# microsoft/msrflute

Hardware: AMD Instinct MI355X
Metric: fl_rounds_per_sec (higher is better)
Workload: dtype fp32; 1 GPU; model=cnn_femnist (2conv+2fc, 62 classes), global_batch=200, seq_len=784, parallelism=client-parallel fedavg, 1 ranks, clients=3400, clients_per_round=10, samples_per_client=200, local_epochs=1, client_batch_size=20, eval_and_checkpoint=outside timed region, precision_detail=fp32 throughout

## Files before the change

msrflute_amd/csrc/bindings.cpp:

```cpp

#include <torch/extension.h>
#include <c10/hip/HIPStream.h>
#include <hip/hip_runtime.h>

#include "launchers.h"

namespace {

hipStream_t cur_stream() {
  return c10::hip::getCurrentHIPStream().stream();
}

void check_flat(const torch::Tensor& t, const char* name) {
  TORCH_CHECK(t.is_cuda(), name, " must be on GPU");
  TORCH_CHECK(t.is_contiguous(), name, " must be contiguous");
  TORCH_CHECK(t.scalar_type() == torch::kFloat32, name, " must be fp32");
}

void pseudo_grad(torch::Tensor out, torch::Tensor ws, torch::Tensor wt,
                 double weight) {
  check_flat(out, "out"); check_flat(ws, "ws"); check_flat(wt, "wt");
  TORCH_CHECK(out.numel() == ws.numel() && ws.numel() == wt.numel());
  launch_pseudo_grad(out.data_ptr<float>(), ws.data_ptr<float>(),
                     wt.data_ptr<float>(), (float)weight, out.numel(),
                     cur_stream());
}

void axpy(torch::Tensor y, torch::Tensor x, double alpha) {
  check_flat(y, "y"); check_flat(x, "x");
  TORCH_CHECK(y.numel() == x.numel());
  launch_axpy(y.data_ptr<float>(), x.data_ptr<float>(), (float)alpha,
              y.numel(), cur_stream());
}

void scale(torch::Tensor x, double alpha) {
  check_flat(x, "x");
  launch_scale(x.data_ptr<float>(), (float)alpha, x.numel(), cur_stream());
}

static torch::Tensor sum_sumsq_acc(const torch::Tensor& x) {
  auto acc = torch::zeros({2}, x.options().dtype(torch::kFloat64));
  int nparts = sum_sumsq2_partials(x.numel());
  auto partials = torch::empty({2 * (long long)nparts},
                               x.options().dtype(torch::kFloat64));
  launch_sum_sumsq2(x.data_ptr<float>(), x.numel(),
                    partials.data_ptr<double>(), acc.data_ptr<double>(),
                    cur_stream());
  return acc;
}

torch::Tensor sum_sumsq(torch::Tensor x) {
  check_flat(x, "x");
  return sum_sumsq_acc(x).to(torch::kFloat32);
}

torch::Tensor clip_by_norm(torch::Tensor x, double max_norm, double eps) {
  check_flat(x, "x");
  auto acc = sum_sumsq_acc(x);
  auto norm = torch::empty({}, x.options());
  launch_clip_apply(x.data_ptr<float>(), x.numel(), acc.data_ptr<double>(),
                    (float)max_norm, (float)eps, norm.data_ptr<float>(),
                    cur_stream());
  return norm;
}

void add_gaussian_noise(torch::Tensor x, double sigma, int64_t seed,
                        int64_t offset) {
  check_flat(x, "x");
  launch_add_gaussian_noise(x.data_ptr<float>(), x.numel(), (float)sigma,
                            (unsigned long long)seed,
                            (unsigned long long)offset, cur_stream());
}

void sgd_step(torch::Tensor p, torch::Tensor g, torch::Tensor buf, double lr,
              double momentum, double dampening, double weight_decay,
              bool nesterov, bool first_step) {
  check_flat(p, "p"); check_flat(g, "g");
  if (momentum != 0.0) {
    check_flat(buf, "buf");
    TORCH_CHECK(buf.numel() == p.numel(), "momentum buffer size mismatch");
  }
  launch_sgd_step(p.data_ptr<float>(), g.data_ptr<float>(),
                  buf.numel() ? buf.data_ptr<float>() : nullptr, (float)lr,
                  nullptr, (float)momentum, (float)dampening,
                  (float)weight_decay, nesterov ? 1 : 0, first_step ? 1 : 0,
                  p.numel(), cur_stream());
}

void sgd_step_devlr(torch::Tensor p, torch::Tensor g, torch::Tensor buf,
                    torch::Tensor lr_t, double momentum, double dampening,
                    double weight_decay, bool nesterov, bool first_step) {
  check_flat(p, "p"); check_flat(g, "g"); check_flat(lr_t, "lr_t");
  if (momentum != 0.0) {
    check_flat(buf, "buf");
    TORCH_CHECK(buf.numel() == p.numel(), "momentum buffer size mismatch");
  }
  launch_sgd_step(p.data_ptr<float>(), g.data_ptr<float>(),
                  buf.numel() ? buf.data_ptr<float>() : nullptr, 0.f,
                  lr_t.data_ptr<float>(), (float)momentum, (float)dampening,
                  (float)weight_decay, nesterov ? 1 : 0, first_step ? 1 : 0,
                  p.numel(), cur_stream());
}

void clip_stats_accumulate(torch::Tensor x, double max_norm, double eps,
                           torch::Tensor stats_acc) {
  check_flat(x, "x"); check_flat(stats_acc, "stats_acc");
  TORCH_CHECK(stats_acc.numel() >= 2, "stats_acc must have 2 elements");
  auto acc = sum_sumsq_acc(x);
  launch_clip_apply_stats(x.data_ptr<float>(), x.numel(),
                          acc.data_ptr<double>(), (float)max_norm, (float)eps,
                          stats_acc.data_ptr<float>(), cur_stream());
}

void adam_step(torch::Tensor p, torch::Tensor g, torch::Tensor m,
               torch::Tensor v, torch::Tensor vmax, int64_t step, double lr,
               double beta1, double beta2, double eps, double weight_decay,
               bool amsgrad, bool adamw) {
  check_flat(p, "p"); check_flat(g, "g"); check_flat(m, "m"); check_flat(v, "v");
  if (amsgrad) check_flat(vmax, "vmax");
  float bc1 = 1.0f - (float)std::pow(beta1, (double)step);
  float bc2 = 1.0f - (float)std::pow(beta2, (double)step);
  launch_adam_step(p.data_ptr<float>(), g.data_ptr<float>(),
                   m.data_ptr<float>(), v.data_ptr<float>(),
                   vmax.numel() ? vmax.data_ptr<float>() : nullptr, (float)lr,
                   (float)beta1, (float)beta2, (float)eps, (float)weight_decay,
                   bc1, bc2, amsgrad ? 1 : 0, adamw ? 1 : 0, p.numel(),
                   cur_stream());
}

void adamax_step(torch::Tensor p, torch::Tensor g, torch::Tensor m,
                 torch::Tensor u, int64_t step, double lr, double beta1,
                 double beta2, double eps, double weight_decay) {
  check_flat(p, "p"); check_flat(g, "g"); check_flat(m, "m"); check_flat(u, "u");
  float bc1 = 1.0f - (float)std::pow(beta1, (double)step);
  launch_adamax_step(p.data_ptr<float>(), g.data_ptr<float>(),
                     m.data_ptr<float>(), u.data_ptr<float>(), (float)lr,
                     (float)beta1, (float)beta2, (float)eps,
                     (float)weight_decay, bc1, p.numel(), cur_stream());
}

torch::Tensor segmented_sqnorm(torch::Tensor x, torch::Tensor seg_offsets) {
  check_flat(x, "x");
  TORCH_CHECK(seg_offsets.is_cuda() && seg_offsets.is_contiguous() &&
              seg_offsets.scalar_type() == torch::kInt64,
              "seg_offsets must be contiguous int64 on GPU");
  int n_segs = (int)seg_offsets.numel() - 1;
  auto out = torch::zeros({n_segs}, x.options().dtype(torch::kFloat64));
  launch_segmented_sqnorm(
      x.data_ptr<float>(),
      reinterpret_cast<const long long*>(seg_offsets.data_ptr<int64_t>()),
      n_segs, out.data_ptr<double>(), cur_stream());
  return out.to(torch::kFloat32);
}

void quant_bin_mask(torch::Tensor x, torch::Tensor min_t, torch::Tensor max_t,
                    torch::Tensor thresh_t, int64_t n_bins) {
  check_flat(x, "x");
  check_flat(min_t, "min_t"); check_flat(max_t, "max_t");
  check_flat(thresh_t, "thresh_t");
  launch_quant_bin_mask(x.data_ptr<float>(), x.numel(),
                        min_t.data_ptr<float>(), max_t.data_ptr<float>(),
                        thresh_t.data_ptr<float>(), (int)n_bins, cur_stream());
}

static CnnWorkspace slice_ws(torch::Tensor& work_f, torch::Tensor& work_i,
                             torch::Tensor& work_b, torch::Tensor& work_d,
                             int B, int C) {
  float* f = work_f.data_ptr<float>();
  CnnWorkspace ws;
  ws.xb = f;            f += (long long)B * 784;
  ws.a1 = f;            f += (long long)B * 21632;
  ws.r2 = f;            f += (long long)B * 36864;
  ws.a2 = f;            f += (long long)B * 9216;
  ws.z3 = f;            f += (long long)B * 128;
  ws.a3 = f;            f += (long long)B * 128;
  ws.dz3 = f;           f += (long long)B * 128;
  ws.da2 = f;           f += (long long)B * 9216;
  ws.dz2 = f;           f += (long long)B * 36864;
  ws.dz1 = f;           f += (long long)B * 21632;
  ws.wsl = f;           f += (long long)B * 18432;
  ws.w2t = f;           f += 18432;
  ws.w2rot = f;         f += 18432;
  ws.dlogits = f;       f += (long long)B * C;
  TORCH_CHECK(f - work_f.data_ptr<float>() <= work_f.numel(),
              "float workspace too small");
  TORCH_CHECK(work_i.numel() >= B, "int workspace too small");
  TORCH_CHECK(work_d.numel() >= 2 * 2048 + 2, "double workspace too small");
  ws.yb = work_i.data_ptr<int>();
  unsigned char* u = work_b.data_ptr<unsigned char>();
  ws.pidx = u;          u += (long long)B * 9216;
  ws.m2 = u;            u += (long long)B * 9216;
  ws.m3 = u;            u += (long long)B * 128;
  TORCH_CHECK(u - work_b.data_ptr<unsigned char>() <= work_b.numel(),
              "byte workspace too small");
  ws.red_partials = work_d.data_ptr<double>();
  ws.red_acc = work_d.data_ptr<double>() + work_d.numel() - 2;
  return ws;
}

void cnn_epoch(torch::Tensor shard_x, torch::Tensor shard_y,
               torch::Tensor order, int64_t bs, int64_t C,
               torch::Tensor params, torch::Tensor grads,
               torch::Tensor work_f, torch::Tensor work_i,
               torch::Tensor work_b, torch::Tensor work_d,
               torch::Tensor lr_t, double max_norm, double p1, double p2,
               torch::Tensor stats_acc, torch::Tensor loss_acc,
               int64_t seed, bool use_bf16) {
  check_flat(params, "params"); check_flat(grads, "grads");
  check_flat(lr_t, "lr_t"); check_flat(stats_acc, "stats_acc");
  check_flat(loss_acc, "loss_acc"); check_flat(work_f, "work_f");
  TORCH_CHECK(shard_x.is_cuda() && shard_x.is_contiguous() &&
              shard_x.scalar_type() == torch::kFloat32, "shard_x");
  TORCH_CHECK(shard_y.is_cuda() && shard_y.is_contiguous() &&
              shard_y.scalar_type() == torch::kInt64, "shard_y");
  TORCH_CHECK(order.is_cuda() && order.scalar_type() == torch::kInt64,
              "order must be int64 on device");
  long long n = shard_y.numel();
  TORCH_CHECK(shard_x.numel() == n * 784, "shard_x must be [n,784]");
  TORCH_CHECK(bs >= 1 && bs <= 32, "fused CNN epoch supports batch <= 32");
  int B = (int)bs;
  CnnWorkspace ws = slice_ws(work_f, work_i, work_b, work_d, B, (int)C);
  launch_cnn_epoch(shard_x.data_ptr<float>(),
                   reinterpret_cast<const long long*>(
                       shard_y.data_ptr<int64_t>()),
                   reinterpret_cast<const long long*>(
                       order.data_ptr<int64_t>()),
                   n, B, (int)C,
                   params.data_ptr<float>(), grads.data_ptr<float>(), ws,
                   lr_t.data_ptr<float>(), (float)max_norm, (float)p1,
                   (float)p2, stats_acc.data_ptr<float>(),
                   loss_acc.data_ptr<float>(), (unsigned long long)seed,
                   cur_stream(), 0, use_bf16 ? 1 : 0);
}

void cnn_round(torch::Tensor shard_x, torch::Tensor shard_y,
               torch::Tensor orders_dev, torch::Tensor row_bases,
               torch::Tensor order_offs, torch::Tensor counts,
               torch::Tensor weights, torch::Tensor seeds, int64_t bs,
               int64_t C, torch::Tensor server_params, torch::Tensor params,
               torch::Tensor grads, torch::Tensor round_accum,
               torch::Tensor work_f, torch::Tensor work_i,
               torch::Tensor work_b, torch::Tensor work_d,
               torch::Tensor lr_t, double max_norm, double p1, double p2,
               torch::Tensor stats_out, torch::Tensor loss_out,
               bool use_bf16) {
  check_flat(server_params, "server_params"); check_flat(params, "params");
  check_flat(grads, "grads"); check_flat(round_accum, "round_accum");
  TORCH_CHECK(orders_dev.is_cuda() && orders_dev.scalar_type() == torch::kInt64);
  TORCH_CHECK(!row_bases.is_cuda() && !order_offs.is_cuda() &&
              !counts.is_cuda() && !weights.is_cuda() && !seeds.is_cuda(),
              "per-client metadata must be host tensors");
  TORCH_CHECK(row_bases.scalar_type() == torch::kInt64 &&
              order_offs.scalar_type() == torch::kInt64 &&
              counts.scalar_type() == torch::kInt64 &&
              seeds.scalar_type() == torch::kInt64 &&
              weights.scalar_type() == torch::kFloat32,
              "metadata dtypes: int64 (weights fp32)");
  TORCH_CHECK(row_bases.is_contiguous() && order_offs.is_contiguous() &&
              counts.is_contiguous() && weights.is_contiguous() &&
              seeds.is_contiguous());
  int K = (int)counts.numel();
  TORCH_CHECK(stats_out.numel() >= 2 * K && loss_out.numel() >= K);
  TORCH_CHECK(bs >= 1 && bs <= 32);
  TORCH_CHECK(row_bases.numel() == K && order_offs.numel() == K &&
              weights.numel() == K && seeds.numel() == K,
              "per-client metadata lengths must all equal K");
  {
    long long n_rows = shard_y.numel();
    TORCH_CHECK(shard_x.numel() == n_rows * 784,
                "shard_x rows must match shard_y (784 features each)");
    long long n_orders = orders_dev.numel();
    auto rb = row_bases.accessor<int64_t, 1>();
    auto oo = order_offs.accessor<int64_t, 1>();
    auto ct = counts.accessor<int64_t, 1>();
    for (int k = 0; k < K; ++k) {
      TORCH_CHECK(ct[k] >= 0 && rb[k] >= 0 && oo[k] >= 0,
                  "negative per-client metadata at k=", k);
      TORCH_CHECK(rb[k] + ct[k] <= n_rows,
                  "client ", k, ": row_base+count ", rb[k] + ct[k],
                  " exceeds shard rows ", n_rows);
      TORCH_CHECK(oo[k] + ct[k] <= n_orders,
                  "client ", k, ": order_off+count ", oo[k] + ct[k],
                  " exceeds orders length ", n_orders);
    }
  }
  CnnWorkspace ws = slice_ws(work_f, work_i, work_b, work_d, (int)bs, (int)C);
  launch_cnn_round(
      shard_x.data_ptr<float>(),
      reinterpret_cast<const long long*>(shard_y.data_ptr<int64_t>()),
      reinterpret_cast<const long long*>(orders_dev.data_ptr<int64_t>()),
      reinterpret_cast<const long long*>(row_bases.data_ptr<int64_t>()),
      reinterpret_cast<const long long*>(order_offs.data_ptr<int64_t>()),
      reinterpret_cast<const long long*>(counts.data_ptr<int64_t>()),
      weights.data_ptr<float>(),
      reinterpret_cast<const unsigned long long*>(seeds.data_ptr<int64_t>()),
      K, (int)bs, (int)C, server_params.data_ptr<float>(),
      params.data_ptr<float>(), grads.data_ptr<float>(),
      round_accum.data_ptr<float>(), ws, lr_t.data_ptr<float>(),
      (float)max_norm, (float)p1, (float)p2, stats_out.data_ptr<float>(),
      loss_out.data_ptr<float>(), cur_stream(), use_bf16 ? 1 : 0);
}

static bool lstm_w_is_bf16(const torch::Tensor& w, const char* layout) {
  if (w.scalar_type() == torch::kFloat32) {
    check_flat(w, "w_packed_stack");
    return false;
  }
  TORCH_CHECK(w.scalar_type() == torch::kBFloat16,
              "w_packed_stack must be float32 or bfloat16");
  TORCH_CHECK(w.is_cuda(), "w_packed_stack must be a GPU tensor");
  TORCH_CHECK(w.is_contiguous(), "w_packed_stack must be contiguous ",
              layout);
  TORCH_CHECK(reinterpret_cast<uintptr_t>(w.data_ptr()) % 16 == 0,
              "w_packed_stack must be 16-byte aligned");
  return true;
}

std::vector<torch::Tensor> lstm_seq_fwd(torch::Tensor xp,
                                        torch::Tensor w_packed_stack,
                                        int64_t rows_per_client) {
  check_flat(xp, "xp");
  bool bf16 = lstm_w_is_bf16(w_packed_stack,
                             "[K, 256/8, 4*256, 8] (ops/lstm._pack_fwd_bf16)");
  TORCH_CHECK(xp.dim() == 3 && xp.size(2) == 4 * 256,
              "fused LSTM supports hidden size 256: xp must be "
              "[R, T, 4*256]");
  long long R = xp.size(0), T = xp.size(1);
  TORCH_CHECK(rows_per_client > 0 && R % rows_per_client == 0);
  long long K = R / rows_per_client;
  TORCH_CHECK(w_packed_stack.numel() == K * 256 * 4 * 256,
              "w_packed_stack must be [K, 256/4, 4*256, 4] "
              "(ops/lstm._pack_fwd)");
  auto h_seq = torch::empty({R, T, 256}, xp.options());
  auto gates = torch::empty({R, T, 4 * 256}, xp.options());
  auto c_seq = torch::empty({R, T, 256}, xp.options());
  if (bf16)
    launch_lstm_seq_fwd_bf16(
        xp.data_ptr<float>(),
        static_cast<const unsigned short*>(w_packed_stack.data_ptr()),
        h_seq.data_ptr<float>(), gates.data_ptr<float>(),
        c_seq.data_ptr<float>(), (int)R, (int)rows_per_client, (int)T,
        cur_stream());
  else
    launch_lstm_seq_fwd(xp.data_ptr<float>(),
                        w_packed_stack.data_ptr<float>(),
                        h_seq.data_ptr<float>(), gates.data_ptr<float>(),
                        c_seq.data_ptr<float>(), (int)R,
                        (int)rows_per_client, (int)T, cur_stream());
  return {h_seq, gates, c_seq};
}

torch::Tensor lstm_seq_bwd(torch::Tensor gates, torch::Tensor c_seq,
                           torch::Tensor w_packed_stack,
                           torch::Tensor dh_out, int64_t rows_per_client) {
  check_flat(gates, "gates"); check_flat(c_seq, "c_seq");
  bool bf16 = lstm_w_is_bf16(w_packed_stack,
                             "[K, 4*256/8, 256, 8] (ops/lstm._pack_bwd_bf16)");
  check_flat(dh_out, "dh_out");
  long long R = gates.size(0), T = gates.size(1);
  TORCH_CHECK(rows_per_client > 0 && R % rows_per_client == 0);
  long long K = R / rows_per_client;
  TORCH_CHECK(w_packed_stack.numel() == K * 4 * 256 * 256,
              "w_packed_stack must be [K, 4*256/4, 256, 4] "
              "(ops/lstm._pack_bwd)");
  auto dg = torch::empty_like(gates);
  if (bf16)
    launch_lstm_seq_bwd_bf16(
        gates.data_ptr<float>(), c_seq.data_ptr<float>(),
        static_cast<const unsigned short*>(w_packed_stack.data_ptr()),
        dh_out.data_ptr<float>(), dg.data_ptr<float>(), (int)R,
        (int)rows_per_client, (int)T, cur_stream());
  else
    launch_lstm_seq_bwd(gates.data_ptr<float>(), c_seq.data_ptr<float>(),
                        w_packed_stack.data_ptr<float>(),
                        dh_out.data_ptr<float>(), dg.data_ptr<float>(),
                        (int)R, (int)rows_per_client, (int)T, cur_stream());
  return dg;
}

std::vector<torch::Tensor> gru_seq_fwd(torch::Tensor gi, torch::Tensor whh_t,
                                       torch::Tensor b_hh) {
  check_flat(gi, "gi"); check_flat(whh_t, "whh_t"); check_flat(b_hh, "b_hh");
  TORCH_CHECK(gi.dim() == 3 && gi.size(2) == 3 * 512 &&
              whh_t.numel() == 512 * 3 * 512,
              "fused GRU supports hidden size 512; pass W_hh "
              "float4-packed [H/4, 3H, 4] (ops/lstm._GRUSeq)");
  long long B = gi.size(0), T = gi.size(1);
  auto h_seq = torch::empty({B, T, 512}, gi.options());
  auto gates = torch::empty({B, T, 3 * 512}, gi.options());
  auto ghn = torch::empty({B, T, 512}, gi.options());
  launch_gru_seq_fwd(gi.data_ptr<float>(), whh_t.data_ptr<float>(),
                     b_hh.data_ptr<float>(), h_seq.data_ptr<float>(),
                     gates.data_ptr<float>(), ghn.data_ptr<float>(),
                     (int)B, (int)T, cur_stream());
  return {h_seq, gates, ghn};
}

std::vector<torch::Tensor> gru_seq_bwd(torch::Tensor gates, torch::Tensor ghn,
                                       torch::Tensor h_seq,
                                       torch::Tensor w_hh,
                                       torch::Tensor dh_out) {
  check_flat(gates, "gates"); check_flat(ghn, "ghn");
  check_flat(h_seq, "h_seq"); check_flat(w_hh, "w_hh");
  check_flat(dh_out, "dh_out");
  TORCH_CHECK(w_hh.numel() == 3 * 512 * 512,
              "gru_seq_bwd wants W_hh float4-packed [3H/4, H, 4]");
  long long B = gates.size(0), T = gates.size(1);
  auto dgi = torch::empty_like(gates);
  auto dgh = torch::empty_like(gates);
  launch_gru_seq_bwd(gates.data_ptr<float>(), ghn.data_ptr<float>(),
                     h_seq.data_ptr<float>(), w_hh.data_ptr<float>(),
                     dh_out.data_ptr<float>(), dgi.data_ptr<float>(),
                     dgh.data_ptr<float>(), (int)B, (int)T, cur_stream());
  return {dgi, dgh};
}

torch::Tensor gru_gates(torch::Tensor g_i, torch::Tensor g_h,
                        torch::Tensor h) {
  check_flat(g_i, "g_i"); check_flat(g_h, "g_h"); check_flat(h, "h");
  int B = (int)h.size(0), H = (int)h.size(1);
  TORCH_CHECK(g_i.numel() == 3LL * B * H && g_h.numel() == 3LL * B * H,
              "g_i/g_h must be [B, 3H]");
  auto out = torch::empty_like(h);
  launch_gru_gates(g_i.data_ptr<float>(), g_h.data_ptr<float>(),
                   h.data_ptr<float>(), out.data_ptr<float>(), B, H,
                   cur_stream());
  return out;
}

}

static int rows_per_client(int64_t B, int64_t K) {
  TORCH_CHECK(K >= 1 && B >= K && B % K == 0, "B rows must split over K");
  return (int)(B / K);
}

static int fc1_rows_per_client(int64_t B, int64_t K) {
  int bs = rows_per_client(B, K);
  TORCH_CHECK(bs <= 32, "fc1 kernels take at most 32 rows per client");
  return bs;
}

static int stack_len(const torch::Tensor& w, int64_t per, const char* name) {
  TORCH_CHECK(w.numel() > 0 && w.numel() % per == 0, name,
              " must hold K blocks of ", per);
  return (int)(w.numel() / per);
}

torch::Tensor dbg_conv2_fwd_mfma(torch::Tensor a1, torch::Tensor w2,
                                 torch::Tensor b2, int64_t B) {
  check_flat(a1, "a1"); check_flat(w2, "w2"); check_flat(b2, "b2");
  int K = stack_len(w2, 18432, "w2");
  int bs = rows_per_client(B, K);
  TORCH_CHECK(a1.numel() >= B * 21632 && b2.numel() == K * 64);
  auto r2 = torch::empty({B * 36864}, a1.options());
  auto w2t = torch::empty_like(w2);
  auto w2rot = torch::empty_like(w2);
  launch_w2_layouts(w2.data_ptr<float>(), K, w2t.data_ptr<float>(),
                    w2rot.data_ptr<float>(), cur_stream());
  launch_conv2_fwd_mfma(a1.data_ptr<float>(), w2t.data_ptr<float>(),
                        b2.data_ptr<float>(), bs, K, r2.data_ptr<float>(),
                        cur_stream());
  return r2;
}

torch::Tensor dbg_conv2_fwd_mfma_bf16(torch::Tensor a1, torch::Tensor w2,
                                      torch::Tensor b2, int64_t B) {
  check_flat(a1, "a1"); check_flat(w2, "w2"); check_flat(b2, "b2");
  int K = stack_len(w2, 18432, "w2");
  int bs = rows_per_client(B, K);
  TORCH_CHECK(a1.numel() >= B * 21632 && b2.numel() == K * 64);
  auto w2b2 = torch::cat({w2.view({K, 18432}), b2.view({K, 64})}, 1)
                  .contiguous();
  auto r2 = torch::empty({B * 36864}, a1.options());
  launch_conv2_fwd_mfma_bf16(a1.data_ptr<float>(), w2b2.data_ptr<float>(),
                             bs, K, r2.data_ptr<float>(), cur_stream());
  return r2;
}

torch::Tensor dbg_conv2_bwd_x_mfma_bf16(torch::Tensor dz2, torch::Tensor w2,
                                        torch::Tensor a1, int64_t B) {
  check_flat(dz2, "dz2"); check_flat(w2, "w2"); check_flat(a1, "a1");
  int K = stack_len(w2, 18432, "w2");
  int bs = rows_per_client(B, K);
  TORCH_CHECK(dz2.numel() >= B * 36864 && a1.numel() >= B * 21632);
  auto dz1 = torch::empty({B * 21632}, dz2.options());
  auto w2rotbf = torch::empty_like(w2);
  launch_conv2_bwd_x_mfma_bf16(dz2.data_ptr<float>(), w2.data_ptr<float>(),
                               a1.data_ptr<float>(), bs, K,
                               w2rotbf.data_ptr<float>(),
                               dz1.data_ptr<float>(), cur_stream());
  return dz1;
}

std::vector<torch::Tensor> dbg_conv2_bwd_w_mfma_bf16(torch::Tensor dz2,
                                                     torch::Tensor a1,
                                                     int64_t B, int64_t K) {
  check_flat(dz2, "dz2"); check_flat(a1, "a1");
  int bs = rows_per_client(B, K);
  TORCH_CHECK(dz2.numel() >= B * 36864 && a1.numel() >= B * 21632);
  auto slab = torch::empty({B * 18432}, dz2.options());
  auto dw2 = torch::empty({K * 18432}, dz2.options());
  auto db2 = torch::empty({K * 64}, dz2.options());
  launch_conv2_bwd_w_mfma_bf16(dz2.data_ptr<float>(), a1.data_ptr<float>(),
                               bs, (int)K, slab.data_ptr<float>(),
                               dw2.data_ptr<float>(), db2.data_ptr<float>(),
                               cur_stream());
  return {dw2, db2};
}

std::vector<torch::Tensor> dbg_fc1_fwd_mfma_bf16(torch::Tensor a2,
                                                 torch::Tensor w3,
                                                 torch::Tensor b3, int64_t B,
                                                 double p2, int64_t seed,
                                                 int64_t offset) {
  check_flat(a2, "a2"); check_flat(w3, "w3"); check_flat(b3, "b3");
  int K = stack_len(w3, 128 * 9216, "w3");
  int bs = fc1_rows_per_client(B, K);
  TORCH_CHECK(a2.numel() >= B * 9216 && b3.numel() == K * 128);
  auto slab = torch::empty({36 * B * 128}, a2.options());
  auto z3 = torch::empty({B * 128}, a2.options());
  auto a3 = torch::empty({B * 128}, a2.options());
  auto m3 = torch::empty({B * 128}, a2.options().dtype(torch::kUInt8));
  launch_fc1_fwd_mfma_bf16(a2.data_ptr<float>(), w3.data_ptr<float>(),
                           b3.data_ptr<float>(), bs, K, (float)p2,
                           (unsigned long long)seed,
                           (unsigned long long)offset,
                           slab.data_ptr<float>(), z3.data_ptr<float>(),
                           a3.data_ptr<float>(), m3.data_ptr<unsigned char>(),
                           cur_stream());
  return {z3, a3, m3};
}

torch::Tensor dbg_conv2_bwd_x_mfma(torch::Tensor dz2, torch::Tensor w2,
                                   torch::Tensor a1, int64_t B) {
  check_flat(dz2, "dz2"); check_flat(w2, "w2"); check_flat(a1, "a1");
  int K = stack_len(w2, 18432, "w2");
  int bs = rows_per_client(B, K);
  TORCH_CHECK(dz2.numel() >= B * 36864 && a1.numel() >= B * 21632);
  auto dz1 = torch::empty({B * 21632}, dz2.options());
  auto w2t = torch::empty_like(w2);
  auto w2rot = torch::empty_like(w2);
  launch_w2_layouts(w2.data_ptr<float>(), K, w2t.data_ptr<float>(),
                    w2rot.data_ptr<float>(), cur_stream());
  launch_conv2_bwd_x_mfma(dz2.data_ptr<float>(), w2rot.data_ptr<float>(),
                          a1.data_ptr<float>(), bs, K,
                          dz1.data_ptr<float>(), cur_stream());
  return dz1;
}

std::vector<torch::Tensor> dbg_conv2_bwd_w_mfma(torch::Tensor dz2,
                                                torch::Tensor a1, int64_t B,
                                                int64_t K) {
  check_flat(dz2, "dz2"); check_flat(a1, "a1");
  int bs = rows_per_client(B, K);
  TORCH_CHECK(dz2.numel() >= B * 36864 && a1.numel() >= B * 21632);
  auto slab = torch::empty({B * 18432}, dz2.options());
  auto dw2 = torch::empty({K * 18432}, dz2.options());
  auto db2 = torch::empty({K * 64}, dz2.options());
  launch_conv2_bwd_w_mfma(dz2.data_ptr<float>(), a1.data_ptr<float>(),
                          bs, (int)K, slab.data_ptr<float>(),
                          dw2.data_ptr<float>(), db2.data_ptr<float>(),
                          cur_stream());
  return {dw2, db2};
}

std::vector<torch::Tensor> dbg_fc1_fwd_mfma(torch::Tensor a2,
                                            torch::Tensor w3,
                                            torch::Tensor b3, int64_t B,
                                            double p2, int64_t seed,
                                            int64_t offset) {
  check_flat(a2, "a2"); check_flat(w3, "w3"); check_flat(b3, "b3");
  int K = stack_len(w3, 128 * 9216, "w3");
  int bs = fc1_rows_per_client(B, K);
  TORCH_CHECK(a2.numel() >= B * 9216 && b3.numel() == K * 128);
  auto slab = torch::empty({64 * B * 128}, a2.options());
  auto z3 = torch::empty({B * 128}, a2.options());
  auto a3 = torch::empty({B * 128}, a2.options());
  auto m3 = torch::empty({B * 128}, a2.options().dtype(torch::kUInt8));
  launch_fc1_fwd_mfma(a2.data_ptr<float>(), w3.data_ptr<float>(),
                      b3.data_ptr<float>(), bs, K, (float)p2,
                      (unsigned long long)seed, (unsigned long long)offset,
                      slab.data_ptr<float>(), z3.data_ptr<float>(),
                      a3.data_ptr<float>(), m3.data_ptr<unsigned char>(),
                      cur_stream());
  return {z3, a3, m3};
}

std::vector<torch::Tensor> dbg_fc1_bwd_w_mfma(torch::Tensor dz3,
                                              torch::Tensor a2, int64_t B,
                                              int64_t K) {
  check_flat(dz3, "dz3"); check_flat(a2, "a2");
  int bs = fc1_rows_per_client(B, K);
  TORCH_CHECK(dz3.numel() >= B * 128 && a2.numel() >= B * 9216);
  auto dw3 = torch::empty({K * 128 * 9216}, dz3.options());
  auto db3 = torch::empty({K * 128}, dz3.options());
  launch_fc1_bwd_w_mfma(dz3.data_ptr<float>(), a2.data_ptr<float>(), bs,
                        (int)K, dw3.data_ptr<float>(), db3.data_ptr<float>(),
                        cur_stream());
  return {dw3, db3};
}

torch::Tensor dbg_fc1_bwd_x_mfma(torch::Tensor dz3, torch::Tensor w3,
                                 int64_t B) {
  check_flat(dz3, "dz3"); check_flat(w3, "w3");
  int K = stack_len(w3, 128 * 9216, "w3");
  int bs = fc1_rows_per_client(B, K);
  TORCH_CHECK(dz3.numel() >= B * 128);
  auto da2 = torch::empty({B * 9216}, dz3.options());
  launch_fc1_bwd_x_mfma(dz3.data_ptr<float>(), w3.data_ptr<float>(), bs, K,
                        da2.data_ptr<float>(), cur_stream());
  return da2;
}

torch::Tensor dbg_mfma_bf16_probe(torch::Tensor A, torch::Tensor B) {
  TORCH_CHECK(A.is_cuda() && A.scalar_type() == torch::kBFloat16 &&
              A.is_contiguous() && A.numel() == 16 * 32);
  TORCH_CHECK(B.is_cuda() && B.scalar_type() == torch::kBFloat16 &&
              B.is_contiguous() && B.numel() == 32 * 16);
  auto D = torch::empty({16, 16},
                        A.options().dtype(torch::kFloat32));
  launch_mfma_bf16_probe(A.data_ptr(), B.data_ptr(), D.data_ptr<float>(),
                         cur_stream());
  return D;
}

void cnn_round_mega(torch::Tensor shard_x, torch::Tensor shard_y,
                    torch::Tensor orders_dev, torch::Tensor row_bases_dev,
                    torch::Tensor order_offs_dev, torch::Tensor counts_dev,
                    torch::Tensor counts_host, torch::Tensor weights_dev,
                    torch::Tensor seeds_dev, int64_t bs, int64_t C,
                    torch::Tensor server_params, torch::Tensor params_stack,
                    torch::Tensor grads_stack, torch::Tensor round_accum,
                    torch::Tensor work_f, torch::Tensor work_i,
                    torch::Tensor work_b, torch::Tensor work_d,
                    torch::Tensor lr_t, double max_norm, double p1,
                    double p2, torch::Tensor stats_out,
                    torch::Tensor loss_out, bool use_bf16) {
  check_flat(server_params, "server_params");
  check_flat(params_stack, "params_stack");
  check_flat(grads_stack, "grads_stack");
  check_flat(round_accum, "round_accum");
  check_flat(work_f, "work_f");
  TORCH_CHECK(orders_dev.is_cuda() && row_bases_dev.is_cuda() &&
              order_offs_dev.is_cuda() && counts_dev.is_cuda() &&
              weights_dev.is_cuda() && seeds_dev.is_cuda(),
              "mega metadata must be device tensors");
  TORCH_CHECK(!counts_host.is_cuda() &&
              counts_host.scalar_type() == torch::kInt64);
  int K = (int)counts_host.numel();
  TORCH_CHECK(row_bases_dev.numel() == K && order_offs_dev.numel() == K &&
              counts_dev.numel() == K && weights_dev.numel() == K &&
              seeds_dev.numel() == K, "metadata lengths must equal K");
  TORCH_CHECK(bs >= 1 && bs <= 32);
  long long P = server_params.numel();
  TORCH_CHECK(params_stack.numel() >= (long long)K * P &&
              grads_stack.numel() >= (long long)K * P,
              "parameter stacks too small");
  TORCH_CHECK(stats_out.numel() >= 2 * K && loss_out.numel() >= K);
  {
    long long n_rows = shard_y.numel();
    long long n_orders = orders_dev.numel();
    auto rb = row_bases_dev.cpu();
    auto oo = order_offs_dev.cpu();
    auto rba = rb.accessor<int64_t, 1>();
    auto ooa = oo.accessor<int64_t, 1>();
    auto ct = counts_host.accessor<int64_t, 1>();
    for (int k = 0; k < K; ++k) {
      TORCH_CHECK(ct[k] > 0 && rba[k] >= 0 && ooa[k] >= 0 &&
                  rba[k] + ct[k] <= n_rows &&
                  ooa[k] + ct[k] <= n_orders,
                  "client ", k, ": metadata out of bounds");
    }
  }
  int G = K * (int)bs;
  float* f = work_f.data_ptr<float>();
  auto take = [&](long long n) { float* p = f; f += n; return p; };
  float* xb = take((long long)G * 784);
  float* a1 = take((long long)G * 21632);
  float* r2 = take((long long)G * 36864);
  float* a2 = take((long long)G * 9216);
  float* z3 = take((long long)G * 128);
  float* a3 = take((long long)G * 128);
  float* dz3 = take((long long)G * 128);
  float* da2 = take((long long)G * 9216);
  float* dz2 = take((long long)G * 36864);
  float* dz1 = take((long long)G * 21632);
  float* w2t = take((long long)K * 18432);
  float* w2rot = take((long long)K * 18432);
  float* slab = take((long long)G * 18432);
  float* dlg = take((long long)G * C);
  TORCH_CHECK(f - work_f.data_ptr<float>() <= work_f.numel(),
              "mega float workspace too small");
  TORCH_CHECK(work_i.numel() >= G, "mega int workspace too small");
  unsigned char* u = work_b.data_ptr<unsigned char>();
  unsigned char* pidx = u;
  unsigned char* m2 = u + (long long)G * 9216;
  unsigned char* m3 = u + (long long)G * 9216 * 2;
  TORCH_CHECK(work_b.numel() >= (long long)G * (9216 * 2 + 128),
              "mega byte workspace too small");
  TORCH_CHECK(work_d.numel() >= 2 * K, "mega double workspace too small");
  launch_cnn_round_mega(
      shard_x.data_ptr<float>(),
      reinterpret_cast<const long long*>(shard_y.data_ptr<int64_t>()),
      reinterpret_cast<const long long*>(orders_dev.data_ptr<int64_t>()),
      reinterpret_cast<const long long*>(row_bases_dev.data_ptr<int64_t>()),
      reinterpret_cast<const long long*>(order_offs_dev.data_ptr<int64_t>()),
      reinterpret_cast<const long long*>(counts_dev.data_ptr<int64_t>()),
      reinterpret_cast<const long long*>(counts_host.data_ptr<int64_t>()),
      weights_dev.data_ptr<float>(),
      reinterpret_cast<const long long*>(seeds_dev.data_ptr<int64_t>()),
      K, (int)bs, (int)C, server_params.data_ptr<float>(),
      params_stack.data_ptr<float>(), grads_stack.data_ptr<float>(),
      round_accum.data_ptr<float>(),
      xb, a1, r2, a2, z3, a3, dlg, dz3, da2, dz2, dz1, w2t, w2rot, slab,
      work_i.data_ptr<int>(), pidx, m2, m3, work_d.data_ptr<double>(),
      lr_t.data_ptr<float>(), (float)max_norm, (float)p1, (float)p2,
      stats_out.data_ptr<float>(), loss_out.data_ptr<float>(),
      cur_stream(), use_bf16 ? 1 : 0);
}

void mega_clip_sgd(torch::Tensor params_stack, torch::Tensor grads_stack,
                   int64_t K, torch::Tensor acc2k, double max_norm,
                   torch::Tensor lr_t, torch::Tensor stats_out) {
  check_flat(params_stack, "params_stack");
  check_flat(grads_stack, "grads_stack");
  check_flat(lr_t, "lr_t"); check_flat(stats_out, "stats_out");
  TORCH_CHECK(K > 0 && params_stack.numel() % K == 0 &&
              params_stack.numel() == grads_stack.numel());
  TORCH_CHECK(acc2k.is_cuda() && acc2k.scalar_type() == torch::kFloat64 &&
              acc2k.numel() >= 2 * K);
  TORCH_CHECK(stats_out.numel() >= 2 * K);
  long long P = params_stack.numel() / K;
  launch_mega_clip_sgd(params_stack.data_ptr<float>(),
                       grads_stack.data_ptr<float>(), P, (int)K,
                       acc2k.data_ptr<double>(), (float)max_norm,
                       lr_t.data_ptr<float>(), stats_out.data_ptr<float>(),
                       cur_stream());
}

void mega_pseudo_accum(torch::Tensor grads_stack, torch::Tensor server,
                       torch::Tensor params_stack, torch::Tensor weights_dev,
                       torch::Tensor round_accum) {
  check_flat(grads_stack, "grads_stack"); check_flat(server, "server");
  check_flat(params_stack, "params_stack");
  check_flat(weights_dev, "weights_dev");
  check_flat(round_accum, "round_accum");
  long long P = server.numel();
  TORCH_CHECK(P > 0 && params_stack.numel() % P == 0);
  int K = (int)(params_stack.numel() / P);
  TORCH_CHECK(weights_dev.numel() >= K && round_accum.numel() == P &&
              grads_stack.numel() == params_stack.numel());
  launch_mega_pseudo_accum(grads_stack.data_ptr<float>(),
                           server.data_ptr<float>(),
                           params_stack.data_ptr<float>(),
                           weights_dev.data_ptr<float>(),
                           round_accum.data_ptr<float>(), P, K,
                           cur_stream());
}

PYBIND11_MODULE(TORCH_EXTENSION_NAME, m) {
  m.attr("CONV2_FWD_SLAB_ROWS") = CONV2_FWD_SLAB_ROWS;
  m.def("cnn_round_mega", &cnn_round_mega);
  m.def("mega_clip_sgd", &mega_clip_sgd);
  m.def("mega_pseudo_accum", &mega_pseudo_accum);
  m.def("dbg_mfma_bf16_probe", &dbg_mfma_bf16_probe);
  m.def("dbg_conv2_fwd_mfma_bf16", &dbg_conv2_fwd_mfma_bf16);
  m.def("dbg_conv2_bwd_x_mfma_bf16", &dbg_conv2_bwd_x_mfma_bf16);
  m.def("dbg_conv2_bwd_w_mfma_bf16", &dbg_conv2_bwd_w_mfma_bf16,
        py::arg("dz2"), py::arg("a1"), py::arg("B"), py::arg("K") = 1);
  m.def("dbg_fc1_fwd_mfma_bf16", &dbg_fc1_fwd_mfma_bf16);
  m.def("dbg_conv2_fwd_mfma", &dbg_conv2_fwd_mfma);
  m.def("dbg_conv2_bwd_x_mfma", &dbg_conv2_bwd_x_mfma);
  m.def("dbg_conv2_bwd_w_mfma", &dbg_conv2_bwd_w_mfma,
        py::arg("dz2"), py::arg("a1"), py::arg("B"), py::arg("K") = 1);
  m.def("dbg_fc1_fwd_mfma", &dbg_fc1_fwd_mfma);
  m.def("dbg_fc1_bwd_w_mfma", &dbg_fc1_bwd_w_mfma,
        py::arg("dz3"), py::arg("a2"), py::arg("B"), py::arg("K") = 1);
  m.def("dbg_fc1_bwd_x_mfma", &dbg_fc1_bwd_x_mfma);
  m.doc() = "msrflute_amd gfx950 flat-arena kernels";
  m.def("pseudo_grad", &pseudo_grad);
  m.def("axpy", &axpy);
  m.def("scale", &scale);
  m.def("sum_sumsq", &sum_sumsq);
  m.def("clip_by_norm", &clip_by_norm);
  m.def("add_gaussian_noise", &add_gaussian_noise);
  m.def("sgd_step", &sgd_step);
  m.def("sgd_step_devlr", &sgd_step_devlr);
  m.def("clip_stats_accumulate", &clip_stats_accumulate);
  m.def("adam_step", &adam_step);
  m.def("adamax_step", &adamax_step);
  m.def("segmented_sqnorm", &segmented_sqnorm);
  m.def("quant_bin_mask", &quant_bin_mask);
  m.def("gru_gates", &gru_gates);
  m.def("cnn_epoch", &cnn_epoch);
  m.def("cnn_round", &cnn_round);
  m.def("lstm_seq_fwd", &lstm_seq_fwd);
  m.def("gru_seq_fwd", &gru_seq_fwd);
  m.def("gru_seq_bwd", &gru_seq_bwd);
  m.def("lstm_seq_bwd", &lstm_seq_bwd);
}
```

msrflute_amd/csrc/fused_cnn.hip:

```cpp

#include <hip/hip_runtime.h>
#include <hiprand/hiprand_kernel.h>

#include <cstdio>
#include <cstdlib>

#include "launchers.h"

#define FBLK 256

typedef __attribute__((ext_vector_type(4))) float f32x4;

__device__ __forceinline__ int mega_Bk(const long long* counts, int k,
                                       int t, int bs) {
  long long rem = counts[k] - (long long)t * bs;
  return rem <= 0 ? 0 : (rem < bs ? (int)rem : bs);
}

__global__ void k_copy_stack(float* __restrict__ dst,
                             const float* __restrict__ src, long long P,
                             int K) {
  long long total = (long long)K * P;
  for (long long i = blockIdx.x * (long long)blockDim.x + threadIdx.x;
       i < total; i += (long long)gridDim.x * blockDim.x)
    dst[i] = src[i % P];
}

__global__ void k_copy(float* __restrict__ dst, const float* __restrict__ src,
                       long long n) {
  for (long long i = blockIdx.x * (long long)blockDim.x + threadIdx.x; i < n;
       i += (long long)gridDim.x * blockDim.x)
    dst[i] = src[i];
}

__global__ void k_cnn_pseudo_grad(float* __restrict__ g,
                                  const float* __restrict__ ws,
                                  const float* __restrict__ wt, float weight,
                                  long long n) {
  for (long long i = blockIdx.x * (long long)blockDim.x + threadIdx.x; i < n;
       i += (long long)gridDim.x * blockDim.x)
    g[i] = (ws[i] - wt[i]) * weight;
}

__global__ void k_cnn_axpy(float* __restrict__ y, const float* __restrict__ x,
                           long long n) {
  for (long long i = blockIdx.x * (long long)blockDim.x + threadIdx.x; i < n;
       i += (long long)gridDim.x * blockDim.x)
    y[i] += x[i];
}

__device__ __forceinline__ void gather_elem(
    const float* __restrict__ shard_x, const long long* __restrict__ shard_y,
    long long src, int j, long long i, long long g,
    float* __restrict__ xb, int* __restrict__ yb) {
  xb[i] = shard_x[src * 784 + j];
  if (j == 0) yb[g] = (int)shard_y[src];
}

__global__ void k_gather_batch(const float* __restrict__ shard_x,
                               const long long* __restrict__ shard_y,
                               const long long* __restrict__ order,
                               long long start, long long row_base, int B,
                               float* __restrict__ xb,
                               int* __restrict__ yb) {
  for (int i = blockIdx.x * blockDim.x + threadIdx.x; i < B * 784;
       i += gridDim.x * blockDim.x) {
    int b = i / 784, j = i % 784;
    gather_elem(shard_x, shard_y, row_base + order[start + b], j, i, b,
                xb, yb);
  }
}

__global__ void k_gather_mb(const float* __restrict__ shard_x,
                            const long long* __restrict__ shard_y,
                            const long long* __restrict__ orders,
                            const long long* __restrict__ row_bases,
                            const long long* __restrict__ order_offs,
                            const long long* __restrict__ counts,
                            int t, int bs, int K,
                            float* __restrict__ xb, int* __restrict__ yb) {
  int G = K * bs;
  for (long long i = blockIdx.x * (long long)blockDim.x + threadIdx.x;
       i < (long long)G * 784; i += (long long)gridDim.x * blockDim.x) {
    int g = (int)(i / 784), j = (int)(i % 784);
    int k = g / bs, b = g % bs;
    int Bk = mega_Bk(counts, k, t, bs);
    if (b < Bk) {
      long long src = row_bases[k]
          + orders[order_offs[k] + (long long)t * bs + b];
      gather_elem(shard_x, shard_y, src, j, i, g, xb, yb);
    } else {
      xb[i] = 0.f;
      if (j == 0) yb[g] = -1;
    }
  }
}

__global__ void k_conv1_fwd_mb(const float* __restrict__ x,
                               const float* __restrict__ params, long long P,
                               long long ow1, long long ob1, int bs, int K,
                               float* __restrict__ a1) {
  long long total = (long long)K * bs * 21632;
  for (long long i = blockIdx.x * (long long)blockDim.x + threadIdx.x;
       i < total; i += (long long)gridDim.x * blockDim.x) {
    int xx = (int)(i % 26), yy = (int)((i / 26) % 26);
    int co = (int)((i / 676) % 32);
    long long g = i / 21632;
    int k = (int)(g / bs);
    const float* w1 = params + (long long)k * P + ow1;
    const float* b1 = params + (long long)k * P + ob1;
    const float* xp = x + g * 784 + yy * 28 + xx;
    const float* wp = w1 + co * 9;
    float acc = b1[co];
    #pragma unroll
    for (int kh = 0; kh < 3; ++kh)
      #pragma unroll
      for (int kw = 0; kw < 3; ++kw)
        acc = fmaf(wp[kh * 3 + kw], xp[kh * 28 + kw], acc);
    a1[i] = acc > 0.f ? acc : 0.f;
  }
}

__global__ void k_w2_layouts_mb(const float* __restrict__ params,
                                long long P, long long ow2, int K,
                                float* __restrict__ w2t_stack,
                                float* __restrict__ w2rot_stack) {
  long long total = (long long)K * 18432;
  for (long long i = blockIdx.x * (long long)blockDim.x + threadIdx.x;
       i < total; i += (long long)gridDim.x * blockDim.x) {
    int k = (int)(i / 18432), r = (int)(i % 18432);
    int co = r / 288, kk = r % 288;
    float v = params[(long long)k * P + ow2 + r];
    w2t_stack[(long long)k * 18432 + kk * 64 + co] = v;
    int rem = kk % 9;
    w2rot_stack[(long long)k * 18432 + ((long long)co * 9 + rem) * 32
                + kk / 9] = v;
  }
}

__device__ __forceinline__ void conv2_tap_offsets(int kc, int cs, int rs,
                                                  int sgn, int off[9]) {
  #pragma unroll
  for (int j = 0; j < 9; ++j) {
    int q = 4 * j + kc, c = q / 9, rem = q % 9;
    off[j] = c * cs + sgn * ((rem / 3) * rs + rem % 3);
  }
}

#define C2F_ROWS CONV2_FWD_SLAB_ROWS
#define C2F_SLABS (24 / C2F_ROWS)
#define C2F_CS ((C2F_ROWS + 2) * 26)
static_assert(24 % C2F_ROWS == 0 && (C2F_ROWS * 24) % 96 == 0 &&
              C2F_CS % 4 == 0 && C2F_CS / 4 <= 64,
              "conv2 fwd slab: 6 m-tiles per block, float4 plane copies");
__global__ __launch_bounds__(256)
void k_conv2_fwd_mfma_mb(const float* __restrict__ a1,
                         const float* __restrict__ w2t_stack,
                         const float* __restrict__ params, long long P,
                         long long ob2, int bs, int K,
                         float* __restrict__ r2) {
  __shared__ __attribute__((aligned(16))) float lds[32 * C2F_CS];
  long long g = blockIdx.x / C2F_SLABS;
  int sl = blockIdx.x % C2F_SLABS;
  int k = (int)(g / bs);
  int lane = threadIdx.x & 63, w = threadIdx.x >> 6;
  const float4* src = reinterpret_cast<const float4*>(
      a1 + g * 21632 + sl * (C2F_ROWS * 26));
  if (lane < C2F_CS / 4)
    for (int ci = w; ci < 32; ci += 4)
      reinterpret_cast<float4*>(lds)[ci * (C2F_CS / 4) + lane] =
          src[ci * 169 + lane];
  __syncthreads();
  int il = lane & 15, kc = lane >> 4;
  int nh = w & 1, mh = w >> 1;
  int off[9], base[3];
  conv2_tap_offsets(kc, C2F_CS, 26, 1, off);
  #pragma unroll
  for (int i = 0; i < 3; ++i) {
    int m = (mh * 3 + i) * 16 + il;
    base[i] = (m / 24) * 26 + m % 24;
  }
  const float* wp = w2t_stack + (long long)k * 18432 + kc * 64 + nh * 32 + il;
  f32x4 acc[3][2];
  #pragma unroll
  for (int i = 0; i < 3; ++i)
    acc[i][0] = acc[i][1] = f32x4{0, 0, 0, 0};
  for (int t = 0; t < 8; ++t) {
    const float* lt = lds + t * 4 * C2F_CS;
    const float* wt = wp + t * 36 * 64;
    #pragma unroll
    for (int j = 0; j < 9; ++j) {
      float b0 = wt[j * 256], b1 = wt[j * 256 + 16];
      #pragma unroll
      for (int i = 0; i < 3; ++i) {
        float a = lt[base[i] + off[j]];
        acc[i][0] =
            __builtin_amdgcn_mfma_f32_16x16x4f32(a, b0, acc[i][0], 0, 0, 0);
        acc[i][1] =
            __builtin_amdgcn_mfma_f32_16x16x4f32(a, b1, acc[i][1], 0, 0, 0);
      }
    }
  }
  const float* b2 = params + (long long)k * P + ob2;
  #pragma unroll
  for (int n = 0; n < 2; ++n) {
    int co = nh * 32 + n * 16 + il;
    float bias = b2[co];
    #pragma unroll
    for (int i = 0; i < 3; ++i) {
      int om = sl * (C2F_ROWS * 24) + (mh * 3 + i) * 16 + kc * 4;
      float4 v;
      v.x = acc[i][n][0] + bias; v.y = acc[i][n][1] + bias;
      v.z = acc[i][n][2] + bias; v.w = acc[i][n][3] + bias;
      v.x = v.x > 0.f ? v.x : 0.f; v.y = v.y > 0.f ? v.y : 0.f;
      v.z = v.z > 0.f ? v.z : 0.f; v.w = v.w > 0.f ? v.w : 0.f;
      *reinterpret_cast<float4*>(r2 + (g * 64 + co) * 576 + om) = v;
    }
  }
}

template <typename Index>
__device__ __forceinline__ void pool_drop_cell(
    const float* __restrict__ base, Index i, Index li, float p1,
    float inv_keep, unsigned long long seed, unsigned long long offset,
    float* __restrict__ a2, unsigned char* __restrict__ pidx,
    unsigned char* __restrict__ m2) {
  float v0 = base[0], v1 = base[1], v2 = base[24], v3 = base[25];
  float m = v0; int idx = 0;
  if (v1 > m) { m = v1; idx = 1; }
  if (v2 > m) { m = v2; idx = 2; }
  if (v3 > m) { m = v3; idx = 3; }
  unsigned char keep = 1;
  if (p1 > 0.f) {
    hiprandStatePhilox4_32_10_t st;
    hiprand_init(seed, (unsigned long long)(li >> 2), offset, &st);
    float4 u = hiprand_uniform4(&st);
    float uu = (li & 3) == 0 ? u.x : (li & 3) == 1 ? u.y
               : (li & 3) == 2 ? u.z : u.w;
    keep = uu >= p1;
  }
  pidx[i] = (unsigned char)idx;
  m2[i] = keep;
  a2[i] = keep ? m * inv_keep : 0.f;
}

__global__ void k_pool_drop_fwd(const float* __restrict__ r2, int B,
                                float p1, unsigned long long seed,
                                unsigned long long offset,
                                float* __restrict__ a2,
                                unsigned char* __restrict__ pidx,
                                unsigned char* __restrict__ m2) {
  int total = B * 64 * 144;
  float inv_keep = (p1 < 1.f) ? 1.f / (1.f - p1) : 0.f;
  for (int i = blockIdx.x * blockDim.x + threadIdx.x; i < total;
       i += gridDim.x * blockDim.x) {
    int px = i % 12, py = (i / 12) % 12, c = (i / 144) % 64, b = i / 9216;
    const float* base =
        r2 + (((long long)b * 64 + c) * 24 + 2 * py) * 24 + 2 * px;
    pool_drop_cell(base, i, i, p1, inv_keep, seed, offset, a2, pidx, m2);
  }
}

__global__ void k_pool_drop_fwd_mb(const float* __restrict__ r2, int bs,
                                   int K, float p1,
                                   const long long* __restrict__ seeds,
                                   unsigned long long offset,
                                   float* __restrict__ a2,
                                   unsigned char* __restrict__ pidx,
                                   unsigned char* __restrict__ m2) {
  long long total = (long long)K * bs * 9216;
  float inv_keep = (p1 < 1.f) ? 1.f / (1.f - p1) : 0.f;
  for (long long i = blockIdx.x * (long long)blockDim.x + threadIdx.x;
       i < total; i += (long long)gridDim.x * blockDim.x) {
    int px = (int)(i % 12), py = (int)((i / 12) % 12);
    int c = (int)((i / 144) % 64);
    long long g = i / 9216;
    int k = (int)(g / bs), b = (int)(g % bs);
    const float* base = r2 + ((g * 64 + c) * 24 + 2 * py) * 24 + 2 * px;
    long long li = (long long)b * 9216 + (i % 9216);
    pool_drop_cell(base, i, li, p1, inv_keep, (unsigned long long)seeds[k],
                   offset, a2, pidx, m2);
  }
}

typedef __attribute__((ext_vector_type(2))) float f32x2;
__device__ __forceinline__ int addr_vec(unsigned long long a) {
  return (a & 15) == 0 ? 4 : ((a & 7) == 0 ? 2 : 1);
}
template <int VEC>
__device__ __forceinline__ void ld_vec(const float* __restrict__ p,
                                       float* v) {
  if (VEC == 4) {
    f32x4 t = *reinterpret_cast<const f32x4*>(p);
    v[0] = t[0]; v[1] = t[1]; v[2] = t[2]; v[3] = t[3];
  } else if (VEC == 2) {
    f32x2 t = *reinterpret_cast<const f32x2*>(p);
    v[0] = t[0]; v[1] = t[1];
  } else {
    v[0] = p[0];
  }
}
template <int VEC>
__device__ __forceinline__ void st_vec(float* __restrict__ p,
                                       const float* v) {
  if (VEC == 4)
    *reinterpret_cast<f32x4*>(p) = f32x4{v[0], v[1], v[2], v[3]};
  else if (VEC == 2)
    *reinterpret_cast<f32x2*>(p) = f32x2{v[0], v[1]};
  else
    p[0] = v[0];
}

#define FC1_SPLIT 64
#define FC1_CH (9216 / FC1_SPLIT)
#define FC1_SUB 48
#define FC1_LD (FC1_SUB + 2)
template <int VEC>
__device__ __forceinline__ void fc1_fwd_body(
    const float* __restrict__ w3, const float* __restrict__ a2k, int bs,
    int k_base, float* lw, float* la, f32x4 (&acc)[2][2]) {
  constexpr int PER_ROW = FC1_SUB / VEC;
  constexpr int NW = 128 * PER_ROW / 256;
  constexpr int A_ITEMS = 32 * PER_ROW;
  constexpr int NA = (A_ITEMS + 255) / 256;
  float rw[NW][VEC], ra[NA][VEC];
  auto fetch = [&](int sub) {
    int kb = k_base + sub * FC1_SUB;
    #pragma unroll
    for (int n = 0; n < NW; ++n) {
      int i = threadIdx.x + n * 256;
      int row = i / PER_ROW, c = i % PER_ROW;
      ld_vec<VEC>(w3 + (row * 9216 + kb + c * VEC), rw[n]);
    }
    #pragma unroll
    for (int n = 0; n < NA; ++n) {
      int i = threadIdx.x + n * 256;
      int bu = i / PER_ROW, c = i % PER_ROW;
      #pragma unroll
      for (int e = 0; e < VEC; ++e) ra[n][e] = 0.f;
      if (i < A_ITEMS && bu < bs)
        ld_vec<VEC>(a2k + (bu * 9216 + kb + c * VEC), ra[n]);
    }
  };
  int lane = threadIdx.x & 63, w = threadIdx.x >> 6;
  int kc = lane >> 4, il = lane & 15;
  fetch(0);
  #pragma unroll 1
  for (int sub = 0; sub < FC1_CH / FC1_SUB; ++sub) {
    #pragma unroll
    for (int n = 0; n < NW; ++n) {
      int i = threadIdx.x + n * 256;
      int row = i / PER_ROW, c = i % PER_ROW;
      #pragma unroll
      for (int e = 0; e < VEC; ++e)
        lw[row * FC1_LD + c * VEC + e] = rw[n][e];
    }
    #pragma unroll
    for (int n = 0; n < NA; ++n) {
      int i = threadIdx.x + n * 256;
      int bu = i / PER_ROW, c = i % PER_ROW;
      if (i < A_ITEMS) {
        #pragma unroll
        for (int e = 0; e < VEC; ++e)
          la[bu * FC1_LD + c * VEC + e] = ra[n][e];
      }
    }
    __syncthreads();
    if (sub + 1 < FC1_CH / FC1_SUB) fetch(sub + 1);
    #pragma unroll 6
    for (int k0 = 0; k0 < FC1_SUB; k0 += 4) {
      int kk = k0 + kc;
      float a0 = lw[(w * 32 + il) * FC1_LD + kk];
      float a1v = lw[(w * 32 + 16 + il) * FC1_LD + kk];
      #pragma unroll
      for (int u = 0; u < 2; ++u) {
        float bv = la[(u * 16 + il) * FC1_LD + kk];
        acc[0][u] = __builtin_amdgcn_mfma_f32_16x16x4f32(a0, bv, acc[0][u], 0, 0, 0);
        acc[1][u] = __builtin_amdgcn_mfma_f32_16x16x4f32(a1v, bv, acc[1][u], 0, 0, 0);
      }
    }
    __syncthreads();
  }
}

__global__ __launch_bounds__(256, 3)
void k_fc1_fwd_mfma_mb(const float* __restrict__ a2,
                       const float* __restrict__ params, long long P,
                       long long ow3, int bs, int K,
                       float* __restrict__ slab) {
  __shared__ float lw[128 * FC1_LD];
  __shared__ float la[32 * FC1_LD];
  int k = blockIdx.x / FC1_SPLIT;
  int s = blockIdx.x % FC1_SPLIT;
  int k_base = s * FC1_CH;
  const float* w3 = params + (long long)k * P + ow3;
  const float* a2k = a2 + (long long)k * bs * 9216;
  f32x4 acc[2][2] = {{f32x4{0,0,0,0}, f32x4{0,0,0,0}},
                     {f32x4{0,0,0,0}, f32x4{0,0,0,0}}};
  int vec = addr_vec((unsigned long long)w3 | (unsigned long long)a2k);
  if (vec == 4) fc1_fwd_body<4>(w3, a2k, bs, k_base, lw, la, acc);
  else if (vec == 2) fc1_fwd_body<2>(w3, a2k, bs, k_base, lw, la, acc);
  else fc1_fwd_body<1>(w3, a2k, bs, k_base, lw, la, acc);
  int lane = threadIdx.x & 63, w = threadIdx.x >> 6;
  int il = lane & 15;
  float* slk = slab + (long long)k * FC1_SPLIT * bs * 128;
  #pragma unroll
  for (int tt = 0; tt < 2; ++tt)
    #pragma unroll
    for (int u = 0; u < 2; ++u) {
      int bu = u * 16 + il;
      if (bu >= bs) continue;
      int j = w * 32 + tt * 16 + (lane >> 4) * 4;
      #pragma unroll
      for (int r = 0; r < 4; ++r)
        slk[((long long)s * bs + bu) * 128 + j + r] = acc[tt][u][r];
    }
}

#define FC1R_BLK 256
#define FC1R_BATCH 64
template <int SPLIT>
__device__ __forceinline__ void fc1_reduce_elem(
    const float* __restrict__ slk, float bias, int bs, int b, int j,
    long long i, long long li, float p2, unsigned long long seed,
    unsigned long long offset, float* __restrict__ z3,
    float* __restrict__ a3, unsigned char* __restrict__ m3) {
  float t = bias;
  #pragma unroll
  for (int s0 = 0; s0 < SPLIT; s0 += FC1R_BATCH) {
    float v[FC1R_BATCH];
    #pragma unroll
    for (int n = 0; n < FC1R_BATCH; ++n)
      if (s0 + n < SPLIT)
        v[n] = slk[((long long)(s0 + n) * bs + b) * 128 + j];
    #pragma unroll
    for (int n = 0; n < FC1R_BATCH; ++n)
      if (s0 + n < SPLIT) t += v[n];
  }
  z3[i] = t;
  float r = t > 0.f ? t : 0.f;
  unsigned char keep = 1;
  if (p2 > 0.f) {
    hiprandStatePhilox4_32_10_t st;
    hiprand_init(seed ^ 0x9e3779b97f4a7c15ull, (unsigned long long)li,
                 offset, &st);
    keep = hiprand_uniform(&st) >= p2;
  }
  m3[i] = keep;
  a3[i] = keep ? r / (1.f - p2) : 0.f;
}

template <int SPLIT>
__device__ __forceinline__ void fc1_reduce_client(
    const float* __restrict__ slab, const float* __restrict__ b3, int B,
    float p2, unsigned long long seed, unsigned long long offset,
    float* __restrict__ z3, float* __restrict__ a3,
    unsigned char* __restrict__ m3) {
  int i = blockIdx.x * blockDim.x + threadIdx.x;
  if (i >= B * 128) return;
  int b = i / 128, j = i % 128;
  fc1_reduce_elem<SPLIT>(slab, b3[j], B, b, j, i, i, p2, seed, offset,
                         z3, a3, m3);
}

template <int SPLIT>
__device__ __forceinline__ void fc1_reduce_stack(
    const float* __restrict__ slab, const float* __restrict__ params,
    long long P, long long ob3, int bs, int K, float p2,
    const long long* __restrict__ seeds, unsigned long long offset,
    float* __restrict__ z3, float* __restrict__ a3,
    unsigned char* __restrict__ m3) {
  long long total = (long long)K * bs * 128;
  for (long long i = blockIdx.x * (long long)blockDim.x + threadIdx.x;
       i < total; i += (long long)gridDim.x * blockDim.x) {
    long long g = i / 128;
    int j = (int)(i % 128);
    int k = (int)(g / bs), b = (int)(g % bs);
    fc1_reduce_elem<SPLIT>(slab + (long long)k * SPLIT * bs * 128,
                           params[(long long)k * P + ob3 + j], bs, b, j, i,
                           (long long)b * 128 + j, p2,
                           (unsigned long long)seeds[k], offset,
                           z3, a3, m3);
  }
}

__global__ __launch_bounds__(FC1R_BLK) void k_fc1_fwd_reduce(const float* __restrict__ slab,
                                 const float* __restrict__ b3, int B,
                                 float p2, unsigned long long seed,
                                 unsigned long long offset,
                                 float* __restrict__ z3,
                                 float* __restrict__ a3,
                                 unsigned char* __restrict__ m3) {
  fc1_reduce_client<FC1_SPLIT>(slab, b3, B, p2, seed, offset, z3, a3, m3);
}

__global__ __launch_bounds__(FC1R_BLK) void k_fc1_fwd_reduce_mb(const float* __restrict__ slab,
                                    const float* __restrict__ params,
                                    long long P, long long ob3, int bs,
                                    int K, float p2,
                                    const long long* __restrict__ seeds,
                                    unsigned long long offset,
                                    float* __restrict__ z3,
                                    float* __restrict__ a3,
                                    unsigned char* __restrict__ m3) {
  fc1_reduce_stack<FC1_SPLIT>(slab, params, P, ob3, bs, K, p2, seeds, offset,
                              z3, a3, m3);
}

__device__ __forceinline__ void fc2_loss_row(
    const float* __restrict__ ap, const float* __restrict__ w4,
    const float* __restrict__ b4, int target, int Bk, int C,
    float* __restrict__ dl, float* __restrict__ loss, float* sm) {
  for (int j = threadIdx.x; j < C; j += blockDim.x) {
    const float* wp = w4 + (long long)j * 128;
    float s = b4[j];
    #pragma unroll 4
    for (int kk = 0; kk < 128; ++kk) s = fmaf(wp[kk], ap[kk], s);
    sm[j] = s;
  }
  __syncthreads();
  if (threadIdx.x == 0) {
    float mx = sm[0];
    for (int j = 1; j < C; ++j) mx = fmaxf(mx, sm[j]);
    float z = 0.f;
    for (int j = 0; j < C; ++j) { sm[j] = __expf(sm[j] - mx); z += sm[j]; }
    float inv = 1.f / z;
    for (int j = 0; j < C; ++j) {
      float p = sm[j] * inv;
      dl[j] = (p - (j == target ? 1.f : 0.f)) / (float)Bk;
    }
    atomicAdd(loss, -__logf(fmaxf(sm[target] * inv, 1e-30f)) / (float)Bk);
  }
}

__global__ void k_fc2_loss_fwd(const float* __restrict__ a3,
                               const float* __restrict__ w4,
                               const float* __restrict__ b4,
                               const int* __restrict__ yb, int B, int C,
                               float* __restrict__ dlogits,
                               float* __restrict__ loss_acc) {
  extern __shared__ float sm[];
  int b = blockIdx.x;
  fc2_loss_row(a3 + (long long)b * 128, w4, b4, yb[b], B, C,
               dlogits + (long long)b * C, loss_acc, sm);
}

__global__ void k_fc2_loss_fwd_mb(const float* __restrict__ a3,
                                  const float* __restrict__ params,
                                  long long P, long long ow4, long long ob4,
                                  const long long* __restrict__ counts,
                                  int t, int bs, int K, int C,
                                  const int* __restrict__ yb,
                                  float* __restrict__ dlogits,
                                  float* __restrict__ loss_out) {
  extern __shared__ float sm[];
  long long g = blockIdx.x;
  int k = (int)(g / bs);
  int target = yb[g];
  if (target < 0) {
    for (int j = threadIdx.x; j < C; j += blockDim.x)
      dlogits[g * C + j] = 0.f;
    return;
  }
  fc2_loss_row(a3 + g * 128, params + (long long)k * P + ow4,
               params + (long long)k * P + ob4, target,
               mega_Bk(counts, k, t, bs), C, dlogits + g * C, loss_out + k,
               sm);
}

__global__ void k_fc2_bwd_w_mb(const float* __restrict__ dlogits,
                               const float* __restrict__ a3,
                               float* __restrict__ grads, long long P,
                               long long ow4, long long ob4, int bs, int K,
                               int C) {
  int per_k = (C * 128 + FBLK - 1) / FBLK;
  int k = blockIdx.x / per_k;
  int i0 = (blockIdx.x % per_k) * FBLK + threadIdx.x;
  if (i0 >= C * 128) return;
  int kk = i0 % 128, j = i0 / 128;
  const float* dlk = dlogits + (long long)k * bs * C;
  const float* a3k = a3 + (long long)k * bs * 128;
  float s = 0.f, sb = 0.f;
  for (int b = 0; b < bs; ++b) {
    float d = dlk[(long long)b * C + j];
    s = fmaf(d, a3k[(long long)b * 128 + kk], s);
    if (kk == 0) sb += d;
  }
  grads[(long long)k * P + ow4 + i0] = s;
  if (kk == 0) grads[(long long)k * P + ob4 + j] = sb;
}

__global__ void k_fc2_bwd_x_mb(const float* __restrict__ dlogits,
                               const float* __restrict__ params, long long P,
                               long long ow4, const float* __restrict__ z3,
                               const unsigned char* __restrict__ m3, int bs,
                               int K, int C, float p2,
                               float* __restrict__ dz3) {
  long long total = (long long)K * bs * 128;
  float inv_keep = 1.f / (1.f - p2);
  for (long long i = blockIdx.x * (long long)blockDim.x + threadIdx.x;
       i < total; i += (long long)gridDim.x * blockDim.x) {
    int kk = (int)(i % 128);
    long long g = i / 128;
    int k = (int)(g / bs);
    const float* w4 = params + (long long)k * P + ow4;
    const float* dl = dlogits + g * C;
    float s = 0.f;
    for (int j = 0; j < C; ++j)
      s = fmaf(dl[j], w4[(long long)j * 128 + kk], s);
    float gg = (p2 > 0.f) ? (m3[i] ? s * inv_keep : 0.f) : s;
    dz3[i] = z3[i] > 0.f ? gg : 0.f;
  }
}

#define FC1B_COL(VEC, g, il) ((g) * 16 * (VEC) + (VEC) * (il))

template <int VEC>
__device__ __forceinline__ void fc1_bwd_w_body(
    const float* __restrict__ dz, const float* __restrict__ a2k,
    float* __restrict__ dw3, int bs, int nblk) {
  int lane = threadIdx.x & 63, w = threadIdx.x >> 6;
  int kc = lane >> 4, il = lane & 15;
  f32x4 acc[2][4] = {{f32x4{0,0,0,0}, f32x4{0,0,0,0}, f32x4{0,0,0,0}, f32x4{0,0,0,0}},
                     {f32x4{0,0,0,0}, f32x4{0,0,0,0}, f32x4{0,0,0,0}, f32x4{0,0,0,0}}};
  for (int k0 = 0; k0 < ((bs + 3) & ~3); k0 += 4) {
    int b = k0 + kc;
    bool kv = b < bs;
    int bl = kv ? b : bs - 1;
    float a0 = dz[bl * 128 + w * 32 + il];
    float a1v = dz[bl * 128 + w * 32 + 16 + il];
    float bv[4];
    #pragma unroll
    for (int g = 0; g < 4 / VEC; ++g)
      ld_vec<VEC>(a2k + (bl * 9216 + nblk * 64 + FC1B_COL(VEC, g, il)),
                  bv + g * VEC);
    if (!kv) {
      a0 = 0.f; a1v = 0.f;
      #pragma unroll
      for (int nt = 0; nt < 4; ++nt) bv[nt] = 0.f;
    }
    #pragma unroll
    for (int nt = 0; nt < 4; ++nt) {
      acc[0][nt] = __builtin_amdgcn_mfma_f32_16x16x4f32(a0, bv[nt], acc[0][nt], 0, 0, 0);
      acc[1][nt] = __builtin_amdgcn_mfma_f32_16x16x4f32(a1v, bv[nt], acc[1][nt], 0, 0, 0);
    }
  }
  #pragma unroll
  for (int tt = 0; tt < 2; ++tt) {
    int j = w * 32 + tt * 16 + (lane >> 4) * 4;
    #pragma unroll
    for (int r = 0; r < 4; ++r)
      #pragma unroll
      for (int g = 0; g < 4 / VEC; ++g) {
        float v[VEC];
        #pragma unroll
        for (int e = 0; e < VEC; ++e) v[e] = acc[tt][g * VEC + e][r];
        st_vec<VEC>(dw3 + ((j + r) * 9216 + nblk * 64 +
                           FC1B_COL(VEC, g, il)), v);
      }
  }
}

__global__ __launch_bounds__(256)
void k_fc1_bwd_w_mfma_mb(const float* __restrict__ dz3,
                         const float* __restrict__ a2,
                         float* gw, long long Pw, long long ow3,
                         float* gb, long long Pb, long long ob3,
                         int bs, int K) {
  int k = blockIdx.x / 144;
  int nblk = blockIdx.x % 144;
  const float* dz = dz3 + (long long)k * bs * 128;
  const float* a2k = a2 + (long long)k * bs * 9216;
  float* dw3 = gw + (long long)k * Pw + ow3;
  int vec = addr_vec((unsigned long long)a2k | (unsigned long long)dw3);
  if (vec == 4) fc1_bwd_w_body<4>(dz, a2k, dw3, bs, nblk);
  else if (vec == 2) fc1_bwd_w_body<2>(dz, a2k, dw3, bs, nblk);
  else fc1_bwd_w_body<1>(dz, a2k, dw3, bs, nblk);
  if (nblk == 0 && threadIdx.x < 128) {
    int j = threadIdx.x;
    float s = 0.f;
    for (int b = 0; b < bs; ++b) s += dz[(long long)b * 128 + j];
    gb[(long long)k * Pb + ob3 + j] = s;
  }
}

#define FC1X_WAVES 2
#define FC1X_GRP 8
#define FC1X_BLKS (9216 / (64 * FC1X_WAVES))
template <int VEC>
__device__ __forceinline__ void fc1_bwd_x_body(
    const float* __restrict__ dz, const float* __restrict__ w3,
    float* __restrict__ da, int bs, int col0) {
  int lane = threadIdx.x & 63;
  int kc = lane >> 4, il = lane & 15;
  f32x4 acc[2][4] = {{f32x4{0,0,0,0}, f32x4{0,0,0,0}, f32x4{0,0,0,0}, f32x4{0,0,0,0}},
                     {f32x4{0,0,0,0}, f32x4{0,0,0,0}, f32x4{0,0,0,0}, f32x4{0,0,0,0}}};
  int r0 = (il < bs ? il : bs - 1) * 128 + kc;
  int r1 = (16 + il < bs ? 16 + il : bs - 1) * 128 + kc;
  #pragma unroll 1
  for (int k0 = 0; k0 < 128; k0 += 4 * FC1X_GRP) {
    float bv[FC1X_GRP][4], av[FC1X_GRP][2];
    #pragma unroll
    for (int u = 0; u < FC1X_GRP; ++u) {
      int j = k0 + 4 * u + kc;
      #pragma unroll
      for (int g = 0; g < 4 / VEC; ++g)
        ld_vec<VEC>(w3 + (j * 9216 + col0 + FC1B_COL(VEC, g, il)),
                    bv[u] + g * VEC);
      av[u][0] = dz[r0 + k0 + 4 * u];
      av[u][1] = dz[r1 + k0 + 4 * u];
    }
    #pragma unroll
    for (int u = 0; u < FC1X_GRP; ++u)
      #pragma unroll
      for (int tt = 0; tt < 2; ++tt) {
        float a = tt * 16 + il < bs ? av[u][tt] : 0.f;
        #pragma unroll
        for (int nt = 0; nt < 4; ++nt)
          acc[tt][nt] = __builtin_amdgcn_mfma_f32_16x16x4f32(a, bv[u][nt], acc[tt][nt], 0, 0, 0);
      }
  }
  #pragma unroll
  for (int tt = 0; tt < 2; ++tt) {
    int bu = tt * 16 + (lane >> 4) * 4;
    #pragma unroll
    for (int r = 0; r < 4; ++r) {
      if (bu + r >= bs) continue;
      #pragma unroll
      for (int g = 0; g < 4 / VEC; ++g) {
        float v[VEC];
        #pragma unroll
        for (int e = 0; e < VEC; ++e) v[e] = acc[tt][g * VEC + e][r];
        st_vec<VEC>(da + ((bu + r) * 9216 + col0 + FC1B_COL(VEC, g, il)),
                    v);
      }
    }
  }
}

__global__ __launch_bounds__(64 * FC1X_WAVES)
void k_fc1_bwd_x_mfma_mb(const float* __restrict__ dz3,
                         const float* __restrict__ params, long long P,
                         long long ow3, int bs, int K,
                         float* __restrict__ da2) {
  int k = blockIdx.x / FC1X_BLKS;
  int nblk = blockIdx.x % FC1X_BLKS;
  const float* dz = dz3 + (long long)k * bs * 128;
  const float* w3 = params + (long long)k * P + ow3;
  float* da = da2 + (long long)k * bs * 9216;
  int col0 = (nblk * FC1X_WAVES + (int)(threadIdx.x >> 6)) * 64;
  int vec = addr_vec((unsigned long long)w3 | (unsigned long long)da);
  if (vec == 4) fc1_bwd_x_body<4>(dz, w3, da, bs, col0);
  else if (vec == 2) fc1_bwd_x_body<2>(dz, w3, da, bs, col0);
  else fc1_bwd_x_body<1>(dz, w3, da, bs, col0);
}

__global__ void k_pool_drop_bwd_mb(const float* __restrict__ da2,
                                   const unsigned char* __restrict__ pidx,
                                   const unsigned char* __restrict__ m2,
                                   const float* __restrict__ r2, int bs,
                                   int K, float p1,
                                   float* __restrict__ dz2) {
  long long total = (long long)K * bs * 9216;
  float inv_keep = (p1 < 1.f) ? 1.f / (1.f - p1) : 0.f;
  for (long long i = blockIdx.x * (long long)blockDim.x + threadIdx.x;
       i < total; i += (long long)gridDim.x * blockDim.x) {
    int px = (int)(i % 12), py = (int)((i / 12) % 12);
    int c = (int)((i / 144) % 64);
    long long g = i / 9216;
    float gg = (p1 > 0.f) ? (m2[i] ? da2[i] * inv_keep : 0.f) : da2[i];
    int idx = pidx[i];
    long long base = ((g * 64 + c) * 24 + 2 * py) * 24 + 2 * px;
    #pragma unroll
    for (int d = 0; d < 4; ++d) {
      long long o = base + (d >> 1) * 24 + (d & 1);
      dz2[o] = (d == idx && r2[o] > 0.f) ? gg : 0.f;
    }
  }
}

#define C2W_ROWS 4
#define C2W_OC (C2W_ROWS * 24)
#define C2W_LD (C2W_OC + 2)
#define C2W_PS ((C2W_ROWS + 2) * 26)
static_assert(24 % C2W_ROWS == 0 && C2W_OC % 32 == 0 && C2W_PS <= 256,
              "conv2 bwd_w chunk: whole rows, whole 128 B row pieces, an a1 "
              "plane in two passes of the 128 threads");
__global__ __launch_bounds__(128)
void k_conv2_bwd_w_mfma_mb(const float* __restrict__ dz2,
                           const float* __restrict__ a1, int bs, int K,
                           float* __restrict__ slab) {
  __shared__ __attribute__((aligned(16))) float dzl[64 * C2W_LD];
  __shared__ float apl[5 * C2W_PS];
  int nb = blockIdx.x % 9;
  long long g = blockIdx.x / 9;
  const float* dzb = dz2 + g * 36864;
  const float* a1b = a1 + g * 21632;
  int lane = threadIdx.x & 63, w = threadIdx.x >> 6;
  int il = lane & 15, kc = lane >> 4;
  int ci0 = nb * 32 / 9;
  int npl = 32 - ci0 < 5 ? 32 - ci0 : 5;
  int aoff[2], boff[2];
  #pragma unroll
  for (int q = 0; q < 2; ++q) {
    aoff[q] = (w * 32 + q * 16 + il) * C2W_LD + kc;
    int n = nb * 32 + q * 16 + il;
    int ci = n / 9, rem = n % 9;
    boff[q] = (ci - ci0) * C2W_PS + (rem / 3) * 26 + rem % 3 + kc;
  }
  f32x4 acc[2][2];
  acc[0][0] = acc[0][1] = acc[1][0] = acc[1][1] = f32x4{0, 0, 0, 0};
  int sub = threadIdx.x & 7, r0 = threadIdx.x >> 3;
  float4 pdz[4][C2W_OC / 32];
  float pa[5][2];
  auto fetch = [&](int c) {
    #pragma unroll
    for (int it = 0; it < 4; ++it) {
      const float4* sp = reinterpret_cast<const float4*>(
          dzb + (r0 + 16 * it) * 576 + c * C2W_OC);
      #pragma unroll
      for (int u = 0; u < C2W_OC / 32; ++u) pdz[it][u] = sp[sub + 8 * u];
    }
    #pragma unroll
    for (int p = 0; p < 5; ++p) {
      const float* sp = a1b + (ci0 + p) * 676 + c * (C2W_ROWS * 26);
      #pragma unroll
      for (int h = 0; h < 2; ++h) {
        int j = threadIdx.x + 128 * h;
        pa[p][h] = (p < npl && j < C2W_PS) ? sp[j] : 0.f;
      }
    }
  };
  fetch(0);
  for (int c = 0; c < 24 / C2W_ROWS; ++c) {
    __syncthreads();
    #pragma unroll
    for (int it = 0; it < 4; ++it) {
      float* dp = dzl + (r0 + 16 * it) * C2W_LD;
      #pragma unroll
      for (int u = 0; u < C2W_OC / 32; ++u) {
        float4 v = pdz[it][u];
        float2* d2 = reinterpret_cast<float2*>(dp + 4 * (sub + 8 * u));
        d2[0] = float2{v.x, v.y};
        d2[1] = float2{v.z, v.w};
      }
    }
    #pragma unroll
    for (int p = 0; p < 5; ++p)
      #pragma unroll
      for (int h = 0; h < 2; ++h) {
        int j = threadIdx.x + 128 * h;
        if (j < C2W_PS) apl[p * C2W_PS + j] = pa[p][h];
      }
    __syncthreads();
    if (c + 1 < 24 / C2W_ROWS) fetch(c + 1);
    #pragma unroll
    for (int y = 0; y < C2W_ROWS; ++y)
      #pragma unroll
      for (int s = 0; s < 6; ++s) {
        float a0 = dzl[aoff[0] + y * 24 + 4 * s];
        float a1v = dzl[aoff[1] + y * 24 + 4 * s];
        float b0 = apl[boff[0] + y * 26 + 4 * s];
        float b1 = apl[boff[1] + y * 26 + 4 * s];
        acc[0][0] =
            __builtin_amdgcn_mfma_f32_16x16x4f32(a0, b0, acc[0][0], 0, 0, 0);
        acc[0][1] =
            __builtin_amdgcn_mfma_f32_16x16x4f32(a0, b1, acc[0][1], 0, 0, 0);
        acc[1][0] =
            __builtin_amdgcn_mfma_f32_16x16x4f32(a1v, b0, acc[1][0], 0, 0, 0);
        acc[1][1] =
            __builtin_amdgcn_mfma_f32_16x16x4f32(a1v, b1, acc[1][1], 0, 0, 0);
      }
  }
  float* out = slab + g * 18432;
  #pragma unroll
  for (int mt = 0; mt < 2; ++mt) {
    int orow = w * 32 + mt * 16 + kc * 4;
    #pragma unroll
    for (int nt = 0; nt < 2; ++nt)
      #pragma unroll
      for (int r = 0; r < 4; ++r)
        out[(orow + r) * 288 + nb * 32 + nt * 16 + il] = acc[mt][nt][r];
  }
}

__global__ void k_conv2_bwd_w_fold_mb(const float* __restrict__ slab,
                                      float* __restrict__ grads, long long P,
                                      long long ow2, int bs, int K) {
  int per_k = (18432 + FBLK - 1) / FBLK;
  int k = blockIdx.x / per_k;
  int i = (blockIdx.x % per_k) * FBLK + threadIdx.x;
  if (i >= 18432) return;
  const float* slk = slab + (long long)k * bs * 18432;
  float s = 0.f;
  for (int b = 0; b < bs; ++b) s += slk[(long long)b * 18432 + i];
  grads[(long long)k * P + ow2 + i] = s;
}

__global__ void k_conv2_bwd_b_mb(const float* __restrict__ dz2,
                                 float* __restrict__ grads, long long P,
                                 long long ob2, int bs, int K) {
  int k = blockIdx.x / 64;
  int co = blockIdx.x % 64;
  const float* dzk = dz2 + (long long)k * bs * 36864;
  float s = 0.f;
  for (int t = threadIdx.x; t < bs * 576; t += blockDim.x) {
    int o = t % 576, b = t / 576;
    s += dzk[((long long)b * 64 + co) * 576 + o];
  }
  for (int d = 32; d > 0; d >>= 1) s += __shfl_down(s, d, 64);
  __shared__ float lds[4];
  if ((threadIdx.x & 63) == 0) lds[threadIdx.x >> 6] = s;
  __syncthreads();
  if (threadIdx.x == 0) {
    float tt = 0.f;
    for (int q = 0; q < (int)blockDim.x / 64; ++q) tt += lds[q];
    grads[(long long)k * P + ob2 + co] = tt;
  }
}

#define C2X_MT 128
#define C2X_BLKS ((676 + C2X_MT - 1) / C2X_MT)
#define C2X_ROWS 8
#define C2X_CS (C2X_ROWS * 28)
static_assert((25 + C2X_MT + 25) / 26 + 2 <= C2X_ROWS,
              "conv2 bwd_x: a block's positions span at most ROWS-2 rows");
__global__ __launch_bounds__(256)
void k_conv2_bwd_x_mfma_mb(const float* __restrict__ dz2,
                           const float* __restrict__ w2rot_stack,
                           const float* __restrict__ a1, int bs, int K,
                           float* __restrict__ dz1) {
  __shared__ __attribute__((aligned(16))) float lds[64 * C2X_CS];
  long long g = blockIdx.x / C2X_BLKS;
  int mb = blockIdx.x % C2X_BLKS;
  int k = (int)(g / bs);
  int m0 = mb * C2X_MT, p0 = m0 / 26;
  const float* dzb = dz2 + g * 36864;
  for (int task = threadIdx.x; task < 64 * C2X_ROWS; task += 256) {
    int co = task / C2X_ROWS, lr = task % C2X_ROWS;
    int y = p0 + lr - 2;
    float4 s[6];
    if (y >= 0 && y < 24) {
      const float4* sp =
          reinterpret_cast<const float4*>(dzb + co * 576 + y * 24);
      #pragma unroll
      for (int u = 0; u < 6; ++u) s[u] = sp[u];
    } else {
      #pragma unroll
      for (int u = 0; u < 6; ++u) s[u] = float4{0.f, 0.f, 0.f, 0.f};
    }
    float4* dp = reinterpret_cast<float4*>(lds + co * C2X_CS + lr * 28);
    dp[0] = float4{0.f, 0.f, s[0].x, s[0].y};
    #pragma unroll
    for (int u = 1; u < 6; ++u)
      dp[u] = float4{s[u - 1].z, s[u - 1].w, s[u].x, s[u].y};
    dp[6] = float4{s[5].z, s[5].w, 0.f, 0.f};
  }
  __syncthreads();
  int lane = threadIdx.x & 63, w = threadIdx.x >> 6;
  int il = lane & 15, kc = lane >> 4;
  int mw = m0 + w * 32;
  if (mw >= 676) return;
  int off[9], base[2];
  conv2_tap_offsets(kc, C2X_CS, 28, -1, off);
  #pragma unroll
  for (int i = 0; i < 2; ++i) {
    int m = mw + i * 16 + il;
    m = m < 676 ? m : 675;
    base[i] = (m / 26 - p0 + 2) * 28 + m % 26 + 2;
  }
  const float* wp = w2rot_stack + (long long)k * 18432 + kc * 32 + il;
  f32x4 acc[2][2];
  acc[0][0] = acc[0][1] = acc[1][0] = acc[1][1] = f32x4{0, 0, 0, 0};
  for (int t = 0; t < 16; ++t) {
    const float* lt = lds + t * 4 * C2X_CS;
    const float* wt = wp + t * 36 * 32;
    #pragma unroll
    for (int j = 0; j < 9; ++j) {
      float b0 = wt[j * 128], b1 = wt[j * 128 + 16];
      #pragma unroll
      for (int i = 0; i < 2; ++i) {
        float a = lt[base[i] + off[j]];
        acc[i][0] =
            __builtin_amdgcn_mfma_f32_16x16x4f32(a, b0, acc[i][0], 0, 0, 0);
        acc[i][1] =
            __builtin_amdgcn_mfma_f32_16x16x4f32(a, b1, acc[i][1], 0, 0, 0);
      }
    }
  }
  #pragma unroll
  for (int i = 0; i < 2; ++i) {
    int om = mw + i * 16 + kc * 4;
    if (om >= 676) continue;
    #pragma unroll
    for (int n = 0; n < 2; ++n) {
      long long o = (g * 32 + n * 16 + il) * 676 + om;
      float4 av = *reinterpret_cast<const float4*>(a1 + o);
      float4 v;
      v.x = av.x > 0.f ? acc[i][n][0] : 0.f;
      v.y = av.y > 0.f ? acc[i][n][1] : 0.f;
      v.z = av.z > 0.f ? acc[i][n][2] : 0.f;
      v.w = av.w > 0.f ? acc[i][n][3] : 0.f;
      *reinterpret_cast<float4*>(dz1 + o) = v;
    }
  }
}

__global__ void k_conv1_bwd_w_mb(const float* __restrict__ x,
                                 const float* __restrict__ dz1,
                                 float* __restrict__ grads, long long P,
                                 long long ow1, long long ob1, int bs,
                                 int K) {
  int k = blockIdx.x / 32;
  int co = blockIdx.x % 32;
  const float* xk = x + (long long)k * bs * 784;
  const float* dzk = dz1 + (long long)k * bs * 21632;
  float acc[9] = {0, 0, 0, 0, 0, 0, 0, 0, 0};
  float accb = 0.f;
  for (int t = threadIdx.x; t < bs * 676; t += blockDim.x) {
    int o = t % 676, b = t / 676;
    int xx = o % 26, yy = o / 26;
    float d = dzk[((long long)b * 32 + co) * 676 + o];
    const float* xp = xk + b * 784 + yy * 28 + xx;
    #pragma unroll
    for (int kh = 0; kh < 3; ++kh)
      #pragma unroll
      for (int kw = 0; kw < 3; ++kw)
        acc[kh * 3 + kw] = fmaf(xp[kh * 28 + kw], d, acc[kh * 3 + kw]);
    accb += d;
  }
  __shared__ float lds[16 * 10];
  int n_waves = blockDim.x / 64;
  int wave = threadIdx.x / 64, lane = threadIdx.x % 64;
  #pragma unroll
  for (int kk = 0; kk < 9; ++kk) {
    float s = acc[kk];
    for (int d = 32; d > 0; d >>= 1) s += __shfl_down(s, d, 64);
    if (lane == 0) lds[wave * 10 + kk] = s;
  }
  float sb = accb;
  for (int d = 32; d > 0; d >>= 1) sb += __shfl_down(sb, d, 64);
  if (lane == 0) lds[wave * 10 + 9] = sb;
  __syncthreads();
  if (threadIdx.x < 9) {
    float s = 0.f;
    for (int w = 0; w < n_waves; ++w) s += lds[w * 10 + threadIdx.x];
    grads[(long long)k * P + ow1 + co * 9 + threadIdx.x] = s;
  }
  if (threadIdx.x == 9) {
    float s = 0.f;
    for (int w = 0; w < n_waves; ++w) s += lds[w * 10 + 9];
    grads[(long long)k * P + ob1 + co] = s;
  }
}

#define SUMSQ_CHUNK 32768
__global__ void k_sumsq_mb(const float* __restrict__ grads, long long P,
                           int blocks_per_k, double* __restrict__ acc) {
  int k = blockIdx.x / blocks_per_k;
  int c = blockIdx.x % blocks_per_k;
  long long lo = (long long)c * SUMSQ_CHUNK;
  long long hi = lo + SUMSQ_CHUNK;
  if (hi > P) hi = P;
  const float* g = grads + (long long)k * P;
  double s0 = 0.0, s1 = 0.0, s2 = 0.0, s3 = 0.0;
  double q0 = 0.0, q1 = 0.0, q2 = 0.0, q3 = 0.0;
  long long i = lo + (long long)threadIdx.x * 4;
  for (; i + 3 < hi; i += (long long)blockDim.x * 4) {
    double a = g[i], b = g[i + 1], cc = g[i + 2], d = g[i + 3];
    s0 += a; q0 += a * a;
    s1 += b; q1 += b * b;
    s2 += cc; q2 += cc * cc;
    s3 += d; q3 += d * d;
  }
  for (long long j = i; j < hi; ++j) {
    double v = (double)g[j];
    s0 += v; q0 += v * v;
  }
  double fs = (s0 + s1) + (s2 + s3);
  double fq = (q0 + q1) + (q2 + q3);
  {
  }
  for (int d = 32; d > 0; d >>= 1) {
    fs += __shfl_down(fs, d, 64);
    fq += __shfl_down(fq, d, 64);
  }
  __shared__ double lds[2 * 4];
  int wave = threadIdx.x >> 6, lane = threadIdx.x & 63;
  if (lane == 0) { lds[2 * wave] = fs; lds[2 * wave + 1] = fq; }
  __syncthreads();
  if (threadIdx.x == 0) {
    double ts = 0.0, tq = 0.0;
    for (int w = 0; w < (int)blockDim.x / 64; ++w) {
      ts += lds[2 * w]; tq += lds[2 * w + 1];
    }
    atomicAdd(acc + 2 * k, ts);
    atomicAdd(acc + 2 * k + 1, tq);
  }
}

__device__ __forceinline__ float clip_scale(const double* __restrict__ acc,
                                            int k, float max_norm,
                                            float eps) {
  float norm = (float)sqrt(acc[2 * k + 1]);
  return (max_norm > 0.f && norm > max_norm) ? max_norm / (norm + eps) : 1.f;
}

template <bool STORE_G>
__global__ void k_clip_sgd_mb(float* __restrict__ params,
                              float* __restrict__ grads, long long P, int K,
                              const double* __restrict__ acc, float max_norm,
                              float eps, const float* __restrict__ lr_t,
                              float* __restrict__ stats_out) {
  long long total = (long long)K * P;
  float lr = lr_t[0];
  long long i = blockIdx.x * (long long)blockDim.x + threadIdx.x;
  if (i >= total) return;
  int k = (int)(i / P);
  long long seg_end = (long long)(k + 1) * P;
  float scale = clip_scale(acc, k, max_norm, eps);
  for (; i < total; i += (long long)gridDim.x * blockDim.x) {
    if (i >= seg_end) {
      k = (int)(i / P);
      seg_end = (long long)(k + 1) * P;
      scale = clip_scale(acc, k, max_norm, eps);
    }
    float gv = grads[i] * scale;
    if constexpr (STORE_G) grads[i] = gv;
    params[i] -= lr * gv;
  }
}

__global__ void k_stats_mb(const double* __restrict__ acc, int K,
                           float max_norm, float eps,
                           float* __restrict__ stats_out) {
  int k = blockIdx.x * blockDim.x + threadIdx.x;
  if (k >= K) return;
  float norm = (float)sqrt(acc[2 * k + 1]);
  float scale = (max_norm > 0.f && norm > max_norm)
                    ? max_norm / (norm + eps) : 1.f;
  stats_out[2 * k] += scale * (float)acc[2 * k];
  stats_out[2 * k + 1] += scale * scale * (float)acc[2 * k + 1];
}

__global__ void k_pseudo_grad_mb(float* __restrict__ grads,
                                 const float* __restrict__ server,
                                 const float* __restrict__ params,
                                 const float* __restrict__ weights,
                                 long long P, int K) {
  long long total = (long long)K * P;
  for (long long i = blockIdx.x * (long long)blockDim.x + threadIdx.x;
       i < total; i += (long long)gridDim.x * blockDim.x) {
    int k = (int)(i / P);
    grads[i] = (server[i % P] - params[i]) * weights[k];
  }
}

__global__ void k_accum_mb(float* __restrict__ round_accum,
                           const float* __restrict__ grads, long long P,
                           int K) {
  for (long long p = blockIdx.x * (long long)blockDim.x + threadIdx.x;
       p < P; p += (long long)gridDim.x * blockDim.x) {
    float s = round_accum[p];
    for (int k = 0; k < K; ++k) s += grads[(long long)k * P + p];
    round_accum[p] = s;
  }
}

typedef __attribute__((ext_vector_type(8))) __bf16 bf16x8;

__device__ __forceinline__ bf16x8 ld_bf16x8(const __bf16* p) {
  return *reinterpret_cast<const bf16x8*>(p);
}

__global__ void k_w2rotbf_mb(const float* __restrict__ params, long long P,
                             long long ow2, int K,
                             __bf16* __restrict__ w2rotbf) {
  long long total = (long long)K * 18432;
  for (long long i = blockIdx.x * (long long)blockDim.x + threadIdx.x;
       i < total; i += (long long)gridDim.x * blockDim.x) {
    int k = (int)(i / 18432), r = (int)(i % 18432);
    int co = r / 288, rem9 = r % 288;
    int ci = rem9 / 9, rem = rem9 % 9;
    w2rotbf[(long long)k * 18432 + (long long)ci * 576 + co * 9 + rem] =
        (__bf16)params[(long long)k * P + ow2 + r];
  }
}

#define MC2_LD 296
__global__ __launch_bounds__(256)
void k_conv2_fwd_mfma_mb_bf16(const float* __restrict__ a1,
                              const float* __restrict__ params, long long P,
                              long long ow2, long long ob2, int bs, int K,
                              float* __restrict__ r2) {
  __shared__ __bf16 imc[64 * MC2_LD];
  __shared__ __bf16 wb[64 * MC2_LD];
  long long g = blockIdx.x / 9;
  int mt = blockIdx.x % 9;
  int k = (int)(g / bs);
  const float* a1b = a1 + g * 21632;
  const float* w2 = params + (long long)k * P + ow2;
  const float* b2 = params + (long long)k * P + ob2;
  for (int i = threadIdx.x; i < 64 * 288; i += 256) {
    int mr = i / 288, kk = i % 288;
    int m = mt * 64 + mr, yy = m / 24, xx = m % 24;
    int ci = kk / 9, rem = kk % 9, kh = rem / 3, kw = rem % 3;
    imc[mr * MC2_LD + kk] = (__bf16)a1b[ci * 676 + (yy + kh) * 26 + xx + kw];
    wb[mr * MC2_LD + kk] = (__bf16)w2[i];
  }
  __syncthreads();
  int lane = threadIdx.x & 63, w = threadIdx.x >> 6;
  int il = lane & 15, kc8 = (lane >> 4) * 8;
  f32x4 acc[4] = {f32x4{0,0,0,0}, f32x4{0,0,0,0},
                  f32x4{0,0,0,0}, f32x4{0,0,0,0}};
  for (int k0 = 0; k0 < 288; k0 += 32) {
    bf16x8 a = ld_bf16x8(&imc[(w * 16 + il) * MC2_LD + k0 + kc8]);
    #pragma unroll
    for (int nt = 0; nt < 4; ++nt) {
      bf16x8 bv = ld_bf16x8(&wb[(nt * 16 + il) * MC2_LD + k0 + kc8]);
      acc[nt] = __builtin_amdgcn_mfma_f32_16x16x32_bf16(a, bv, acc[nt], 0, 0, 0);
    }
  }
  int om = mt * 64 + w * 16 + (lane >> 4) * 4;
  #pragma unroll
  for (int r = 0; r < 4; ++r)
    #pragma unroll
    for (int nt = 0; nt < 4; ++nt) {
      int co = nt * 16 + il;
      float v = acc[nt][r] + b2[co];
      r2[(g * 64 + co) * 576 + om + r] = v > 0.f ? v : 0.f;
    }
}

#define MC2B_LD 584
__global__ __launch_bounds__(256)
void k_conv2_bwd_x_mfma_mb_bf16(const float* __restrict__ dz2,
                                const __bf16* __restrict__ w2rotbf,
                                int bs, int K,
                                const float* __restrict__ a1,
                                float* __restrict__ dz1) {
  __shared__ __bf16 imc[32 * MC2B_LD];
  long long g = blockIdx.x / 22;
  int mt = blockIdx.x % 22;
  int k = (int)(g / bs);
  const float* dzb = dz2 + g * 36864;
  const __bf16* wtk = w2rotbf + (long long)k * 18432;
  for (int i = threadIdx.x; i < 32 * 576; i += 256) {
    int mr = i / 576, kk = i % 576;
    int m = mt * 32 + mr, p = m / 26, q = m % 26;
    int co = kk / 9, rem = kk % 9, kh = rem / 3, kw = rem % 3;
    int y = p - kh, x = q - kw;
    imc[mr * MC2B_LD + kk] =
        (__bf16)((m < 676 && y >= 0 && y < 24 && x >= 0 && x < 24)
                     ? dzb[co * 576 + y * 24 + x] : 0.f);
  }
  __syncthreads();
  int lane = threadIdx.x & 63, w = threadIdx.x >> 6;
  int il = lane & 15, kc8 = (lane >> 4) * 8;
  int msub = w & 1, nt = w >> 1;
  f32x4 acc = {0, 0, 0, 0};
  #pragma unroll 3
  for (int k0 = 0; k0 < 576; k0 += 32) {
    bf16x8 a = ld_bf16x8(&imc[(msub * 16 + il) * MC2B_LD + k0 + kc8]);
    bf16x8 bv = ld_bf16x8(&wtk[(long long)(nt * 16 + il) * 576
                                 + k0 + kc8]);
    acc = __builtin_amdgcn_mfma_f32_16x16x32_bf16(a, bv, acc, 0, 0, 0);
  }
  int om = mt * 32 + msub * 16 + (lane >> 4) * 4;
  int ci = nt * 16 + il;
  #pragma unroll
  for (int r = 0; r < 4; ++r) {
    if (om + r >= 676) continue;
    long long o = (g * 32 + ci) * 676 + om + r;
    dz1[o] = a1[o] > 0.f ? acc[r] : 0.f;
  }
}

__global__ __launch_bounds__(256)
void k_conv2_bwd_w_mfma_mb_bf16(const float* __restrict__ dz2,
                                const float* __restrict__ a1, int bs, int K,
                                float* __restrict__ slab) {
  __shared__ __bf16 dzb16[32 * MC2B_LD];
  __shared__ __bf16 imt[32 * MC2B_LD];
  int blk = blockIdx.x % 18;
  int ch = blk / 9;
  int nb = blk % 9;
  long long g = blockIdx.x / 18;
  const float* dzb = dz2 + g * 36864 + (long long)ch * 32 * 576;
  const float* a1b = a1 + g * 21632;
  for (int i = threadIdx.x; i < 32 * 576; i += 256) {
    int co = i / 576;
    dzb16[co * MC2B_LD + (i % 576)] = (__bf16)dzb[i];
  }
  for (int i = threadIdx.x; i < 32 * 576; i += 256) {
    int nr = i / 576, o = i % 576;
    int n = nb * 32 + nr;
    int ci = n / 9, rem = n % 9, kh = rem / 3, kw = rem % 3;
    int yy = o / 24, xx = o % 24;
    imt[nr * MC2B_LD + o] = (__bf16)a1b[ci * 676 + (yy + kh) * 26 + xx + kw];
  }
  __syncthreads();
  int lane = threadIdx.x & 63, w = threadIdx.x >> 6;
  int il = lane & 15, kc8 = (lane >> 4) * 8;
  int csub = w & 1, nt = w >> 1;
  f32x4 acc = {0, 0, 0, 0};
  #pragma unroll 3
  for (int k0 = 0; k0 < 576; k0 += 32) {
    bf16x8 a = ld_bf16x8(&dzb16[(csub * 16 + il) * MC2B_LD + k0 + kc8]);
    bf16x8 bv = ld_bf16x8(&imt[(nt * 16 + il) * MC2B_LD + k0 + kc8]);
    acc = __builtin_amdgcn_mfma_f32_16x16x32_bf16(a, bv, acc, 0, 0, 0);
  }
  float* out = slab + g * 18432;
  int orow = ch * 32 + csub * 16 + (lane >> 4) * 4;
  #pragma unroll
  for (int r = 0; r < 4; ++r)
    out[(orow + r) * 288 + nb * 32 + nt * 16 + il] = acc[r];
}

#define FC1B_SPLIT 36
#define FC1B_CH 256
#define FC1B_LD 264
__global__ __launch_bounds__(256)
void k_fc1_fwd_mfma_mb_bf16(const float* __restrict__ a2,
                            const float* __restrict__ params, long long P,
                            long long ow3, int bs, int K,
                            float* __restrict__ slab) {
  __shared__ __bf16 lw[128 * FC1B_LD];
  __shared__ __bf16 la[32 * FC1B_LD];
  int k = blockIdx.x / FC1B_SPLIT;
  int s = blockIdx.x % FC1B_SPLIT;
  int k_base = s * FC1B_CH;
  const float* w3 = params + (long long)k * P + ow3;
  const float* a2k = a2 + (long long)k * bs * 9216;
  for (int i = threadIdx.x; i < 128 * FC1B_CH; i += 256) {
    int row = i / FC1B_CH, kk = i % FC1B_CH;
    lw[row * FC1B_LD + kk] = (__bf16)w3[(long long)row * 9216 + k_base + kk];
  }
  for (int i = threadIdx.x; i < 32 * FC1B_CH; i += 256) {
    int bu = i / FC1B_CH, kk = i % FC1B_CH;
    la[bu * FC1B_LD + kk] =
        (__bf16)(bu < bs ? a2k[(long long)bu * 9216 + k_base + kk] : 0.f);
  }
  __syncthreads();
  int lane = threadIdx.x & 63, w = threadIdx.x >> 6;
  int il = lane & 15, kc8 = (lane >> 4) * 8;
  f32x4 acc[2][2] = {{f32x4{0,0,0,0}, f32x4{0,0,0,0}},
                     {f32x4{0,0,0,0}, f32x4{0,0,0,0}}};
  for (int k0 = 0; k0 < FC1B_CH; k0 += 32) {
    bf16x8 a0 = ld_bf16x8(&lw[(w * 32 + il) * FC1B_LD + k0 + kc8]);
    bf16x8 a1v = ld_bf16x8(&lw[(w * 32 + 16 + il) * FC1B_LD + k0 + kc8]);
    #pragma unroll
    for (int u = 0; u < 2; ++u) {
      bf16x8 bv = ld_bf16x8(&la[(u * 16 + il) * FC1B_LD + k0 + kc8]);
      acc[0][u] = __builtin_amdgcn_mfma_f32_16x16x32_bf16(a0, bv, acc[0][u], 0, 0, 0);
      acc[1][u] = __builtin_amdgcn_mfma_f32_16x16x32_bf16(a1v, bv, acc[1][u], 0, 0, 0);
    }
  }
  float* slk = slab + (long long)k * FC1B_SPLIT * bs * 128;
  #pragma unroll
  for (int tt = 0; tt < 2; ++tt)
    #pragma unroll
    for (int u = 0; u < 2; ++u) {
      int bu = u * 16 + il;
      if (bu >= bs) continue;
      int j = w * 32 + tt * 16 + (lane >> 4) * 4;
      #pragma unroll
      for (int r = 0; r < 4; ++r)
        slk[((long long)s * bs + bu) * 128 + j + r] = acc[tt][u][r];
    }
}

__global__ __launch_bounds__(FC1R_BLK) void k_fc1_fwd_reduce_bf16(const float* __restrict__ slab,
                                      const float* __restrict__ b3, int B,
                                      float p2, unsigned long long seed,
                                      unsigned long long offset,
                                      float* __restrict__ z3,
                                      float* __restrict__ a3,
                                      unsigned char* __restrict__ m3) {
  fc1_reduce_client<FC1B_SPLIT>(slab, b3, B, p2, seed, offset, z3, a3, m3);
}

__global__ __launch_bounds__(FC1R_BLK) void k_fc1_fwd_reduce_mb_bf16(const float* __restrict__ slab,
                                         const float* __restrict__ params,
                                         long long P, long long ob3, int bs,
                                         int K, float p2,
                                         const long long* __restrict__ seeds,
                                         unsigned long long offset,
                                         float* __restrict__ z3,
                                         float* __restrict__ a3,
                                         unsigned char* __restrict__ m3) {
  fc1_reduce_stack<FC1B_SPLIT>(slab, params, P, ob3, bs, K, p2, seeds,
                               offset, z3, a3, m3);
}

__global__ void k_mfma_bf16_probe(const __bf16* __restrict__ A,
                                  const __bf16* __restrict__ B,
                                  float* __restrict__ D) {
  int l = threadIdx.x;
  bf16x8 a, b;
  #pragma unroll
  for (int e = 0; e < 8; ++e) {
    int k = (l >> 4) * 8 + e;
    a[e] = A[(l & 15) * 32 + k];
    b[e] = B[k * 16 + (l & 15)];
  }
  f32x4 acc = {0, 0, 0, 0};
  acc = __builtin_amdgcn_mfma_f32_16x16x32_bf16(a, b, acc, 0, 0, 0);
  #pragma unroll
  for (int r = 0; r < 4; ++r)
    D[((l >> 4) * 4 + r) * 16 + (l & 15)] = acc[r];
}



#define EPOCH_CHK(name)                                                    \
  do {                                                                     \
    if (epoch_dbg) {                                                       \
      hipError_t e_ = hipStreamSynchronize(s);                             \
      hipError_t e2_ = hipGetLastError();                                  \
      if (e_ != hipSuccess || e2_ != hipSuccess) {                         \
        fprintf(stderr, "cnn_epoch fault after %s (it=%d B=%d): %s / %s\n",\
                name, it, B, hipGetErrorString(e_), hipGetErrorString(e2_));\
        fflush(stderr);                                                    \
        abort();                                                           \
      }                                                                    \
    }                                                                      \
  } while (0)

extern "C" void launch_cnn_epoch(
    const float* shard_x, const long long* shard_y, const long long* order,
    long long n, int bs, int C, float* params, float* grads,
    CnnWorkspace ws, const float* lr_t, float max_norm, float p1, float p2,
    float* stats_acc, float* loss_acc, unsigned long long seed,
    hipStream_t s, long long row_base, int use_bf16) {
  static const bool epoch_dbg = getenv("CNN_EPOCH_DEBUG") != nullptr;
  CnnOffsets o = cnn_offsets(C);
  long long P = o.total;
  const int K = 1;
  int n_batches = (int)((n + bs - 1) / bs);
  for (int it = 0; it < n_batches; ++it) {
    long long start = (long long)it * bs;
    int B = (int)((start + bs <= n) ? bs : (n - start));
    unsigned long long off = (unsigned long long)it;
    hipLaunchKernelGGL(k_gather_batch, dim3((B * 784 + FBLK - 1) / FBLK),
                       dim3(FBLK), 0, s, shard_x, shard_y, order, start,
                       row_base, B, ws.xb, ws.yb);
    EPOCH_CHK("k_gather_batch");
    hipLaunchKernelGGL(k_conv1_fwd_mb, dim3((B * 21632 + FBLK - 1) / FBLK),
                       dim3(FBLK), 0, s, ws.xb, params, P, o.w1, o.b1, B, K,
                       ws.a1);
    EPOCH_CHK("k_conv1_fwd_mb");
    if (use_bf16) {
      hipLaunchKernelGGL(k_w2rotbf_mb, dim3((18432 + FBLK - 1) / FBLK),
                         dim3(FBLK), 0, s, params, P, o.w2, K,
                         reinterpret_cast<__bf16*>(ws.w2rot));
      EPOCH_CHK("k_w2rotbf_mb");
      hipLaunchKernelGGL(k_conv2_fwd_mfma_mb_bf16, dim3(B * 9), dim3(FBLK),
                         0, s, ws.a1, params, P, o.w2, o.b2, B, K, ws.r2);
    } else {
      hipLaunchKernelGGL(k_w2_layouts_mb, dim3((18432 + FBLK - 1) / FBLK),
                         dim3(FBLK), 0, s, params, P, o.w2, K, ws.w2t,
                         ws.w2rot);
      EPOCH_CHK("k_w2_layouts_mb");
      hipLaunchKernelGGL(k_conv2_fwd_mfma_mb, dim3(B * C2F_SLABS),
                         dim3(FBLK), 0, s, ws.a1, ws.w2t, params, P, o.b2, B, K, ws.r2);
    }
    EPOCH_CHK("k_conv2_fwd_mfma_mb");
    hipLaunchKernelGGL(k_pool_drop_fwd, dim3((B * 9216 + FBLK - 1) / FBLK),
                       dim3(FBLK), 0, s, ws.r2, B, p1, seed, off, ws.a2,
                       ws.pidx, ws.m2);
    EPOCH_CHK("k_pool_drop_fwd");
    if (use_bf16) {
      hipLaunchKernelGGL(k_fc1_fwd_mfma_mb_bf16, dim3(FC1B_SPLIT), dim3(FBLK),
                         0, s, ws.a2, params, P, o.w3, B, K, ws.wsl);
      EPOCH_CHK("k_fc1_fwd_mfma_mb_bf16");
      hipLaunchKernelGGL(k_fc1_fwd_reduce_bf16,
                         dim3((B * 128 + FC1R_BLK - 1) / FC1R_BLK),
                         dim3(FC1R_BLK), 0, s, ws.wsl, params + o.b3, B, p2, seed,
                         off, ws.z3, ws.a3, ws.m3);
    } else {
      hipLaunchKernelGGL(k_fc1_fwd_mfma_mb, dim3(FC1_SPLIT), dim3(FBLK), 0, s,
                         ws.a2, params, P, o.w3, B, K, ws.wsl);
      EPOCH_CHK("k_fc1_fwd_mfma_mb");
      hipLaunchKernelGGL(k_fc1_fwd_reduce,
                         dim3((B * 128 + FC1R_BLK - 1) / FC1R_BLK),
                         dim3(FC1R_BLK), 0, s, ws.wsl, params + o.b3, B, p2, seed,
                         off, ws.z3, ws.a3, ws.m3);
    }
    EPOCH_CHK("k_fc1_fwd_reduce");
    hipLaunchKernelGGL(k_fc2_loss_fwd, dim3(B), dim3(FBLK),
                       C * (int)sizeof(float), s, ws.a3, params + o.w4,
                       params + o.b4, ws.yb, B, C, ws.dlogits, loss_acc);
    EPOCH_CHK("k_fc2_loss_fwd");
    hipLaunchKernelGGL(k_fc2_bwd_w_mb, dim3((C * 128 + FBLK - 1) / FBLK),
                       dim3(FBLK), 0, s, ws.dlogits, ws.a3, grads, P, o.w4,
                       o.b4, B, K, C);
    EPOCH_CHK("k_fc2_bwd_w_mb");
    hipLaunchKernelGGL(k_fc2_bwd_x_mb, dim3((B * 128 + FBLK - 1) / FBLK),
                       dim3(FBLK), 0, s, ws.dlogits, params, P, o.w4, ws.z3,
                       ws.m3, B, K, C, p2, ws.dz3);
    EPOCH_CHK("k_fc2_bwd_x_mb");
    hipLaunchKernelGGL(k_fc1_bwd_w_mfma_mb, dim3(144), dim3(FBLK), 0, s,
                       ws.dz3, ws.a2, grads, P, o.w3, grads, P, o.b3, B, K);
    EPOCH_CHK("k_fc1_bwd_w_mfma_mb");
    hipLaunchKernelGGL(k_fc1_bwd_x_mfma_mb, dim3(FC1X_BLKS),
                       dim3(64 * FC1X_WAVES), 0, s,
                       ws.dz3, params, P, o.w3, B, K, ws.da2);
    EPOCH_CHK("k_fc1_bwd_x_mfma_mb");
    hipLaunchKernelGGL(k_pool_drop_bwd_mb, dim3((B * 9216 + FBLK - 1) / FBLK),
                       dim3(FBLK), 0, s, ws.da2, ws.pidx, ws.m2, ws.r2, B, K,
                       p1, ws.dz2);
    EPOCH_CHK("k_pool_drop_bwd_mb");
    if (use_bf16) {
      hipLaunchKernelGGL(k_conv2_bwd_w_mfma_mb_bf16, dim3(18 * B), dim3(FBLK),
                         0, s, ws.dz2, ws.a1, B, K, ws.wsl);
    } else {
      hipLaunchKernelGGL(k_conv2_bwd_w_mfma_mb, dim3(9 * B), dim3(128), 0,
                         s, ws.dz2, ws.a1, B, K, ws.wsl);
    }
    EPOCH_CHK("k_conv2_bwd_w_mfma_mb");
    hipLaunchKernelGGL(k_conv2_bwd_w_fold_mb, dim3((18432 + FBLK - 1) / FBLK),
                       dim3(FBLK), 0, s, ws.wsl, grads, P, o.w2, B, K);
    EPOCH_CHK("k_conv2_bwd_w_fold_mb");
    hipLaunchKernelGGL(k_conv2_bwd_b_mb, dim3(64), dim3(FBLK), 0, s,
                       ws.dz2, grads, P, o.b2, B, K);
    EPOCH_CHK("k_conv2_bwd_b_mb");
    if (use_bf16)
      hipLaunchKernelGGL(k_conv2_bwd_x_mfma_mb_bf16, dim3(B * 22), dim3(FBLK),
                         0, s, ws.dz2,
                         reinterpret_cast<const __bf16*>(ws.w2rot), B, K,
                         ws.a1, ws.dz1);
    else
      hipLaunchKernelGGL(k_conv2_bwd_x_mfma_mb, dim3(B * C2X_BLKS),
                         dim3(FBLK), 0, s, ws.dz2, ws.w2rot, ws.a1, B, K,
                         ws.dz1);
    EPOCH_CHK("k_conv2_bwd_x_mfma_mb");
    hipLaunchKernelGGL(k_conv1_bwd_w_mb, dim3(32), dim3(1024), 0, s,
                       ws.xb, ws.dz1, grads, P, o.w1, o.b1, B, K);
    EPOCH_CHK("k_conv1_bwd_w_mb");
    hipMemsetAsync(ws.red_acc, 0, 2 * sizeof(double), s);
    launch_sum_sumsq2(grads, o.total, ws.red_partials, ws.red_acc, s);
    EPOCH_CHK("launch_sum_sumsq2");
    launch_clip_apply_stats(grads, o.total, ws.red_acc, max_norm, 1e-6f,
                            stats_acc, s);
    EPOCH_CHK("launch_clip_apply_stats");
    launch_sgd_step(params, grads, nullptr, 0.f, lr_t, 0.f, 0.f, 0.f, 0, 0,
                    o.total, s);
    EPOCH_CHK("launch_sgd_step");
  }
}

extern "C" void launch_cnn_round(
    const float* shard_x, const long long* shard_y, const long long* orders,
    const long long* row_bases, const long long* order_offs,
    const long long* counts, const float* weights,
    const unsigned long long* seeds, int K, int bs, int C,
    const float* server_params, float* params, float* grads,
    float* round_accum, CnnWorkspace ws, const float* lr_t, float max_norm,
    float p1, float p2, float* stats_out, float* loss_out,
    hipStream_t s, int use_bf16) {
  CnnOffsets o = cnn_offsets(C);
  int gp = (int)((o.total + FBLK - 1) / FBLK);
  if (gp > 2048) gp = 2048;
  for (int k = 0; k < K; ++k) {
    hipLaunchKernelGGL(k_copy, dim3(gp), dim3(FBLK), 0, s,
                       params, server_params, o.total);
    launch_cnn_epoch(shard_x, shard_y, orders + order_offs[k], counts[k],
                     bs, C, params, grads, ws, lr_t, max_norm, p1, p2,
                     stats_out + 2 * k, loss_out + k, seeds[k], s,
                     row_bases[k], use_bf16);
    hipLaunchKernelGGL(k_cnn_pseudo_grad, dim3(gp), dim3(FBLK), 0, s,
                       grads, server_params, params, weights[k], o.total);
    hipLaunchKernelGGL(k_cnn_axpy, dim3(gp), dim3(FBLK), 0, s,
                       round_accum, grads, o.total);
  }
}

extern "C" void launch_cnn_round_mega(
    const float* shard_x, const long long* shard_y,
    const long long* orders_dev,
    const long long* row_bases_dev, const long long* order_offs_dev,
    const long long* counts_dev, const long long* counts_host,
    const float* weights_dev, const long long* seeds_dev,
    int K, int bs, int C,
    const float* server_params, float* params_stack, float* grads_stack,
    float* round_accum,
    float* xb, float* a1, float* r2, float* a2, float* z3, float* a3,
    float* dlogits, float* dz3, float* da2, float* dz2, float* dz1,
    float* w2t_stack, float* w2rot_stack, float* slab,
    int* yb, unsigned char* pidx, unsigned char* m2, unsigned char* m3,
    double* acc2k,
    const float* lr_t, float max_norm, float p1, float p2,
    float* stats_out, float* loss_out, hipStream_t s, int use_bf16) {
  CnnOffsets o = cnn_offsets(C);
  long long P = o.total;
  int G = K * bs;
  int max_batches = 0;
  for (int k = 0; k < K; ++k) {
    int nb = (int)((counts_host[k] + bs - 1) / bs);
    if (nb > max_batches) max_batches = nb;
  }
  long long kp = (long long)K * P;
  int gkp = (int)((kp + FBLK - 1) / FBLK); if (gkp > 4096) gkp = 4096;
  int gp = (int)((P + FBLK - 1) / FBLK); if (gp > 2048) gp = 2048;
  hipLaunchKernelGGL(k_copy_stack, dim3(gkp), dim3(FBLK), 0, s,
                     params_stack, server_params, P, K);
  for (int t = 0; t < max_batches; ++t) {
    unsigned long long off = (unsigned long long)t;
    hipLaunchKernelGGL(k_gather_mb, dim3((G * 784 + FBLK - 1) / FBLK),
                       dim3(FBLK), 0, s, shard_x, shard_y, orders_dev,
                       row_bases_dev, order_offs_dev, counts_dev, t, bs, K,
                       xb, yb);
    hipLaunchKernelGGL(k_conv1_fwd_mb,
                       dim3((int)(((long long)G * 21632 + FBLK - 1) / FBLK)),
                       dim3(FBLK), 0, s, xb, params_stack, P, o.w1, o.b1,
                       bs, K, a1);
    if (use_bf16) {
      hipLaunchKernelGGL(k_w2rotbf_mb,
                         dim3((int)(((long long)K * 18432 + FBLK - 1) / FBLK)),
                         dim3(FBLK), 0, s, params_stack, P, o.w2, K,
                         reinterpret_cast<__bf16*>(w2rot_stack));
      hipLaunchKernelGGL(k_conv2_fwd_mfma_mb_bf16, dim3(G * 9), dim3(FBLK),
                         0, s, a1, params_stack, P, o.w2, o.b2, bs, K, r2);
    } else {
      hipLaunchKernelGGL(k_w2_layouts_mb,
                         dim3((int)(((long long)K * 18432 + FBLK - 1) / FBLK)),
                         dim3(FBLK), 0, s, params_stack, P, o.w2, K,
                         w2t_stack, w2rot_stack);
      hipLaunchKernelGGL(k_conv2_fwd_mfma_mb, dim3(G * C2F_SLABS),
                         dim3(FBLK), 0, s, a1, w2t_stack, params_stack, P, o.b2, bs, K, r2);
    }
    hipLaunchKernelGGL(k_pool_drop_fwd_mb,
                       dim3((int)(((long long)G * 9216 + FBLK - 1) / FBLK)),
                       dim3(FBLK), 0, s, r2, bs, K, p1, seeds_dev, off,
                       a2, pidx, m2);
    if (use_bf16) {
      hipLaunchKernelGGL(k_fc1_fwd_mfma_mb_bf16, dim3(K * 36), dim3(FBLK),
                         0, s, a2, params_stack, P, o.w3, bs, K, slab);
      hipLaunchKernelGGL(k_fc1_fwd_reduce_mb_bf16,
                         dim3((int)(((long long)G * 128 + FC1R_BLK - 1) /
                                    FC1R_BLK)),
                         dim3(FC1R_BLK), 0, s, slab, params_stack, P, o.b3, bs,
                         K, p2, seeds_dev, off, z3, a3, m3);
    } else {
      hipLaunchKernelGGL(k_fc1_fwd_mfma_mb, dim3(K * FC1_SPLIT), dim3(FBLK),
                         0, s, a2, params_stack, P, o.w3, bs, K, slab);
      hipLaunchKernelGGL(k_fc1_fwd_reduce_mb,
                         dim3((int)(((long long)G * 128 + FC1R_BLK - 1) /
                                    FC1R_BLK)),
                         dim3(FC1R_BLK), 0, s, slab, params_stack, P, o.b3, bs,
                         K, p2, seeds_dev, off, z3, a3, m3);
    }
    hipLaunchKernelGGL(k_fc2_loss_fwd_mb, dim3(G), dim3(FBLK),
                       C * (int)sizeof(float), s, a3, params_stack, P, o.w4,
                       o.b4, counts_dev, t, bs, K, C, yb, dlogits, loss_out);
    int perk_fc2 = (C * 128 + FBLK - 1) / FBLK;
    hipLaunchKernelGGL(k_fc2_bwd_w_mb, dim3(K * perk_fc2), dim3(FBLK), 0, s,
                       dlogits, a3, grads_stack, P, o.w4, o.b4, bs, K, C);
    hipLaunchKernelGGL(k_fc2_bwd_x_mb,
                       dim3((int)(((long long)G * 128 + FBLK - 1) / FBLK)),
                       dim3(FBLK), 0, s, dlogits, params_stack, P, o.w4,
                       z3, m3, bs, K, C, p2, dz3);
    hipLaunchKernelGGL(k_fc1_bwd_w_mfma_mb, dim3(K * 144), dim3(FBLK), 0, s,
                       dz3, a2, grads_stack, P, o.w3, grads_stack, P, o.b3,
                       bs, K);
    hipLaunchKernelGGL(k_fc1_bwd_x_mfma_mb, dim3(K * FC1X_BLKS),
                       dim3(64 * FC1X_WAVES), 0, s,
                       dz3, params_stack, P, o.w3, bs, K, da2);
    hipLaunchKernelGGL(k_pool_drop_bwd_mb,
                       dim3((int)(((long long)G * 9216 + FBLK - 1) / FBLK)),
                       dim3(FBLK), 0, s, da2, pidx, m2, r2, bs, K, p1, dz2);
    if (use_bf16) {
      hipLaunchKernelGGL(k_conv2_bwd_w_mfma_mb_bf16, dim3(18 * G), dim3(FBLK),
                         0, s, dz2, a1, bs, K, slab);
    } else {
      hipLaunchKernelGGL(k_conv2_bwd_w_mfma_mb, dim3(9 * G), dim3(128),
                         0, s, dz2, a1, bs, K, slab);
    }
    int perk_fold = (18432 + FBLK - 1) / FBLK;
    hipLaunchKernelGGL(k_conv2_bwd_w_fold_mb, dim3(K * perk_fold),
                       dim3(FBLK), 0, s, slab, grads_stack, P, o.w2, bs, K);
    hipLaunchKernelGGL(k_conv2_bwd_b_mb, dim3(K * 64), dim3(FBLK), 0, s,
                       dz2, grads_stack, P, o.b2, bs, K);
    if (use_bf16)
      hipLaunchKernelGGL(k_conv2_bwd_x_mfma_mb_bf16, dim3(G * 22), dim3(FBLK),
                         0, s, dz2,
                         reinterpret_cast<const __bf16*>(w2rot_stack),
                         bs, K, a1, dz1);
    else
      hipLaunchKernelGGL(k_conv2_bwd_x_mfma_mb, dim3(G * C2X_BLKS),
                         dim3(FBLK), 0, s, dz2, w2rot_stack, a1, bs, K, dz1);
    hipLaunchKernelGGL(k_conv1_bwd_w_mb, dim3(K * 32), dim3(1024), 0, s,
                       xb, dz1, grads_stack, P, o.w1, o.b1, bs, K);
    hipMemsetAsync(acc2k, 0, 2 * K * sizeof(double), s);
    int blocks_per_k = (int)((P + SUMSQ_CHUNK - 1) / SUMSQ_CHUNK);
    hipLaunchKernelGGL(k_sumsq_mb, dim3(K * blocks_per_k), dim3(FBLK), 0, s,
                       grads_stack, P, blocks_per_k, acc2k);
    hipLaunchKernelGGL(k_stats_mb, dim3((K + 63) / 64), dim3(64), 0, s,
                       acc2k, K, max_norm, 1e-6f, stats_out);
    hipLaunchKernelGGL(k_clip_sgd_mb<false>, dim3(gkp), dim3(FBLK), 0, s,
                       params_stack, grads_stack, P, K, acc2k, max_norm,
                       1e-6f, lr_t, stats_out);
  }
  hipLaunchKernelGGL(k_pseudo_grad_mb, dim3(gkp), dim3(FBLK), 0, s,
                     grads_stack, server_params, params_stack, weights_dev,
                     P, K);
  hipLaunchKernelGGL(k_accum_mb, dim3(gp), dim3(FBLK), 0, s,
                     round_accum, grads_stack, P, K);
}


extern "C" void launch_mega_clip_sgd(float* params_stack, float* grads_stack,
                                     long long P, int K, double* acc2k,
                                     float max_norm, const float* lr_t,
                                     float* stats_out, hipStream_t s) {
  hipMemsetAsync(acc2k, 0, 2 * K * sizeof(double), s);
  int blocks_per_k = (int)((P + SUMSQ_CHUNK - 1) / SUMSQ_CHUNK);
  hipLaunchKernelGGL(k_sumsq_mb, dim3(K * blocks_per_k), dim3(FBLK), 0, s,
                     grads_stack, P, blocks_per_k, acc2k);
  hipLaunchKernelGGL(k_stats_mb, dim3((K + 63) / 64), dim3(64), 0, s,
                     acc2k, K, max_norm, 1e-6f, stats_out);
  long long kp = (long long)K * P;
  int gkp = (int)((kp + FBLK - 1) / FBLK); if (gkp > 4096) gkp = 4096;
  hipLaunchKernelGGL(k_clip_sgd_mb<true>, dim3(gkp), dim3(FBLK), 0, s,
                     params_stack, grads_stack, P, K, acc2k, max_norm,
                     1e-6f, lr_t, stats_out);
}

extern "C" void launch_mega_pseudo_accum(float* grads_stack,
                                         const float* server,
                                         const float* params_stack,
                                         const float* weights_dev,
                                         float* round_accum, long long P,
                                         int K, hipStream_t s) {
  long long kp = (long long)K * P;
  int gkp = (int)((kp + FBLK - 1) / FBLK); if (gkp > 4096) gkp = 4096;
  int gp = (int)((P + FBLK - 1) / FBLK); if (gp > 2048) gp = 2048;
  hipLaunchKernelGGL(k_pseudo_grad_mb, dim3(gkp), dim3(FBLK), 0, s,
                     grads_stack, server, params_stack, weights_dev, P, K);
  hipLaunchKernelGGL(k_accum_mb, dim3(gp), dim3(FBLK), 0, s,
                     round_accum, grads_stack, P, K);
}

#define W2N 18432LL
#define W3N 1179648LL

extern "C" {
void launch_w2_layouts(const float* w2, int K, float* w2t, float* w2rot,
                       hipStream_t s) {
  hipLaunchKernelGGL(k_w2_layouts_mb, dim3((K * 18432 + FBLK - 1) / FBLK),
                     dim3(FBLK), 0, s, w2, W2N, 0LL, K, w2t, w2rot);
}
void launch_conv2_fwd_mfma(const float* a1, const float* w2t, const float* b2,
                           int bs, int K, float* r2, hipStream_t s) {
  hipLaunchKernelGGL(k_conv2_fwd_mfma_mb, dim3(K * bs * C2F_SLABS),
                     dim3(FBLK), 0, s, a1, w2t, b2, 64LL, 0LL, bs, K, r2);
}
void launch_conv2_bwd_x_mfma(const float* dz2, const float* w2rot,
                             const float* a1, int bs, int K, float* dz1,
                             hipStream_t s) {
  hipLaunchKernelGGL(k_conv2_bwd_x_mfma_mb, dim3(K * bs * C2X_BLKS),
                     dim3(FBLK), 0, s, dz2, w2rot, a1, bs, K, dz1);
}
static void conv2_bwd_w_tail(const float* dz2, const float* slab, int bs,
                             int K, float* dw2, float* db2, hipStream_t s) {
  hipLaunchKernelGGL(k_conv2_bwd_w_fold_mb,
                     dim3(K * ((18432 + FBLK - 1) / FBLK)), dim3(FBLK), 0, s,
                     slab, dw2, W2N, 0LL, bs, K);
  hipLaunchKernelGGL(k_conv2_bwd_b_mb, dim3(K * 64), dim3(FBLK), 0, s,
                     dz2, db2, 64LL, 0LL, bs, K);
}
void launch_conv2_bwd_w_mfma(const float* dz2, const float* a1, int bs, int K,
                             float* slab, float* dw2, float* db2,
                             hipStream_t s) {
  hipLaunchKernelGGL(k_conv2_bwd_w_mfma_mb, dim3(9 * K * bs), dim3(128), 0,
                     s, dz2, a1, bs, K, slab);
  conv2_bwd_w_tail(dz2, slab, bs, K, dw2, db2, s);
}
void launch_fc1_fwd_mfma(const float* a2, const float* w3, const float* b3,
                         int bs, int K, float p2, unsigned long long seed,
                         unsigned long long offset, float* slab, float* z3,
                         float* a3, unsigned char* m3, hipStream_t s) {
  hipLaunchKernelGGL(k_fc1_fwd_mfma_mb, dim3(K * FC1_SPLIT), dim3(FBLK), 0, s,
                     a2, w3, W3N, 0LL, bs, K, slab);
  for (int k = 0; k < K; ++k)
    hipLaunchKernelGGL(k_fc1_fwd_reduce,
                       dim3((bs * 128 + FC1R_BLK - 1) / FC1R_BLK),
                       dim3(FC1R_BLK), 0, s,
                       slab + (long long)k * FC1_SPLIT * bs * 128,
                       b3 + k * 128, bs, p2, seed, offset,
                       z3 + k * bs * 128, a3 + k * bs * 128,
                       m3 + k * bs * 128);
}
void launch_fc1_bwd_w_mfma(const float* dz3, const float* a2, int bs, int K,
                           float* dw3, float* db3, hipStream_t s) {
  hipLaunchKernelGGL(k_fc1_bwd_w_mfma_mb, dim3(K * 144), dim3(FBLK), 0, s,
                     dz3, a2, dw3, W3N, 0LL, db3, 128LL, 0LL, bs, K);
}
void launch_fc1_bwd_x_mfma(const float* dz3, const float* w3, int bs, int K,
                           float* da2, hipStream_t s) {
  hipLaunchKernelGGL(k_fc1_bwd_x_mfma_mb, dim3(K * FC1X_BLKS),
                     dim3(64 * FC1X_WAVES), 0, s,
                     dz3, w3, W3N, 0LL, bs, K, da2);
}
void launch_mfma_bf16_probe(const void* A, const void* B, float* D,
                            hipStream_t s) {
  hipLaunchKernelGGL(k_mfma_bf16_probe, dim3(1), dim3(64), 0, s,
                     (const __bf16*)A, (const __bf16*)B, D);
}
void launch_fc1_fwd_mfma_bf16(const float* a2, const float* w3,
                              const float* b3, int bs, int K, float p2,
                              unsigned long long seed,
                              unsigned long long offset, float* slab,
                              float* z3, float* a3, unsigned char* m3,
                              hipStream_t s) {
  hipLaunchKernelGGL(k_fc1_fwd_mfma_mb_bf16, dim3(K * FC1B_SPLIT), dim3(FBLK),
                     0, s, a2, w3, W3N, 0LL, bs, K, slab);
  for (int k = 0; k < K; ++k)
    hipLaunchKernelGGL(k_fc1_fwd_reduce_bf16,
                       dim3((bs * 128 + FC1R_BLK - 1) / FC1R_BLK),
                       dim3(FC1R_BLK), 0, s,
                       slab + (long long)k * FC1B_SPLIT * bs * 128,
                       b3 + k * 128, bs, p2, seed, offset,
                       z3 + k * bs * 128, a3 + k * bs * 128,
                       m3 + k * bs * 128);
}
void launch_conv2_fwd_mfma_bf16(const float* a1, const float* w2b2, int bs,
                                int K, float* r2, hipStream_t s) {
  hipLaunchKernelGGL(k_conv2_fwd_mfma_mb_bf16, dim3(K * bs * 9), dim3(FBLK),
                     0, s, a1, w2b2, W2N + 64, 0LL, W2N, bs, K, r2);
}
void launch_conv2_bwd_x_mfma_bf16(const float* dz2, const float* w2,
                                  const float* a1, int bs, int K,
                                  float* w2rotbf, float* dz1, hipStream_t s) {
  hipLaunchKernelGGL(k_w2rotbf_mb, dim3((K * 18432 + FBLK - 1) / FBLK),
                     dim3(FBLK), 0, s, w2, W2N, 0LL, K,
                     reinterpret_cast<__bf16*>(w2rotbf));
  hipLaunchKernelGGL(k_conv2_bwd_x_mfma_mb_bf16, dim3(K * bs * 22),
                     dim3(FBLK), 0, s, dz2,
                     reinterpret_cast<const __bf16*>(w2rotbf), bs, K, a1,
                     dz1);
}
void launch_conv2_bwd_w_mfma_bf16(const float* dz2, const float* a1, int bs,
                                  int K, float* slab, float* dw2, float* db2,
                                  hipStream_t s) {
  hipLaunchKernelGGL(k_conv2_bwd_w_mfma_mb_bf16, dim3(18 * K * bs),
                     dim3(FBLK), 0, s, dz2, a1, bs, K, slab);
  conv2_bwd_w_tail(dz2, slab, bs, K, dw2, db2, s);
}
}
```

msrflute_amd/csrc/launchers.h:

```cpp
#pragma once

#include <hip/hip_runtime.h>

struct CnnOffsets {
  long long w1, b1, w2, b2, w3, b3, w4, b4, total;
};

inline CnnOffsets cnn_offsets(int C) {
  CnnOffsets o;
  o.w1 = 0;
  o.b1 = o.w1 + 288;
  o.w2 = o.b1 + 32;
  o.b2 = o.w2 + 18432;
  o.w3 = o.b2 + 64;
  o.b3 = o.w3 + 1179648;
  o.w4 = o.b3 + 128;
  o.b4 = o.w4 + (long long)C * 128;
  o.total = o.b4 + C;
  return o;
}

#define CONV2_FWD_SLAB_ROWS 4

struct CnnWorkspace {
  float *xb, *a1, *r2, *a2, *z3, *a3, *dlogits, *dz3, *da2, *dz2, *dz1;
  float *wsl;
  float *w2t, *w2rot;
  int *yb;
  unsigned char *pidx, *m2, *m3;
  double *red_partials, *red_acc;
};

extern "C" {

void launch_pseudo_grad(float* out, const float* ws, const float* wt,
                        float weight, long long n, hipStream_t s);
void launch_axpy(float* y, const float* x, float alpha, long long n,
                 hipStream_t s);
void launch_scale(float* x, float alpha, long long n, hipStream_t s);
void launch_sum_sumsq(const float* x, long long n, double* out2,
                      hipStream_t s);
void launch_sum_sumsq2(const float* x, long long n, double* partials,
                       double* out2, hipStream_t s);
int sum_sumsq2_partials(long long n);
void launch_clip_apply(float* x, long long n, const double* out2,
                       float max_norm, float eps, float* norm_out,
                       hipStream_t s);
void launch_add_gaussian_noise(float* x, long long n, float sigma,
                               unsigned long long seed,
                               unsigned long long offset, hipStream_t s);
void launch_sgd_step(float* p, const float* g, float* buf, float lr,
                     const float* lr_ptr, float momentum, float dampening,
                     float weight_decay, int nesterov, int first_step,
                     long long n, hipStream_t s);
void launch_clip_apply_stats(float* x, long long n, const double* out2,
                             float max_norm, float eps, float* stats_acc,
                             hipStream_t s);
void launch_adam_step(float* p, const float* g, float* m, float* v,
                      float* vmax, float lr, float beta1, float beta2,
                      float eps, float weight_decay, float bc1, float bc2,
                      int amsgrad, int adamw, long long n, hipStream_t s);
void launch_adamax_step(float* p, const float* g, float* m, float* u,
                        float lr, float beta1, float beta2, float eps,
                        float weight_decay, float bc1, long long n,
                        hipStream_t s);
void launch_segmented_sqnorm(const float* x, const long long* offs,
                             int n_segs, double* out, hipStream_t s);
void launch_quant_bin_mask(float* x, long long n, const float* min_t,
                           const float* max_t, const float* thresh_t,
                           int n_bins, hipStream_t s);
void launch_gru_gates(const float* g_i, const float* g_h, const float* h,
                      float* out, int B, int H, hipStream_t s);

void launch_lstm_seq_fwd(const float* xp, const float* w_hh_t_stack,
                         float* h_seq, float* gates, float* c_seq, int R,
                         int rows_per_client, int T, hipStream_t s);
void launch_lstm_seq_bwd(const float* gates, const float* c_seq,
                         const float* w_hh_stack, const float* dh_out,
                         float* dg_pre, int R, int rows_per_client, int T,
                         hipStream_t s);
void launch_lstm_seq_fwd_bf16(const float* xp,
                              const unsigned short* w_hh_t_stack,
                              float* h_seq, float* gates, float* c_seq,
                              int R, int rows_per_client, int T,
                              hipStream_t s);
void launch_lstm_seq_bwd_bf16(const float* gates, const float* c_seq,
                              const unsigned short* w_hh_stack,
                              const float* dh_out, float* dg_pre, int R,
                              int rows_per_client, int T, hipStream_t s);

void launch_gru_seq_fwd(const float* gi, const float* whh_t,
                        const float* b_hh, float* h_seq, float* gates,
                        float* ghn, int B, int T, hipStream_t s);
void launch_gru_seq_bwd(const float* gates, const float* ghn,
                        const float* h_seq, const float* w_hh,
                        const float* dh_out, float* dgi, float* dgh,
                        int B, int T, hipStream_t s);

void launch_cnn_epoch(
    const float* shard_x, const long long* shard_y, const long long* order,
    long long n, int bs, int C, float* params, float* grads,
    CnnWorkspace ws, const float* lr_t, float max_norm, float p1, float p2,
    float* stats_acc, float* loss_acc, unsigned long long seed,
    hipStream_t s, long long row_base, int use_bf16);
void launch_cnn_round(
    const float* shard_x, const long long* shard_y,
    const long long* orders,
    const long long* row_bases,
    const long long* order_offs,
    const long long* counts,
    const float* weights,
    const unsigned long long* seeds,
    int K, int bs, int C,
    const float* server_params, float* params, float* grads,
    float* round_accum, CnnWorkspace ws, const float* lr_t, float max_norm,
    float p1, float p2, float* stats_out, float* loss_out,
    hipStream_t s, int use_bf16);
void launch_cnn_round_mega(
    const float* shard_x, const long long* shard_y,
    const long long* orders_dev,
    const long long* row_bases_dev, const long long* order_offs_dev,
    const long long* counts_dev, const long long* counts_host,
    const float* weights_dev, const long long* seeds_dev,
    int K, int bs, int C,
    const float* server_params, float* params_stack, float* grads_stack,
    float* round_accum,
    float* xb, float* a1, float* r2, float* a2, float* z3, float* a3,
    float* dlogits, float* dz3, float* da2, float* dz2, float* dz1,
    float* w2t_stack, float* w2rot_stack, float* slab,
    int* yb, unsigned char* pidx, unsigned char* m2, unsigned char* m3,
    double* acc2k,
    const float* lr_t, float max_norm, float p1, float p2,
    float* stats_out, float* loss_out, hipStream_t s, int use_bf16);
void launch_mega_clip_sgd(float* params_stack, float* grads_stack,
                          long long P, int K, double* acc2k, float max_norm,
                          const float* lr_t, float* stats_out, hipStream_t s);
void launch_mega_pseudo_accum(float* grads_stack, const float* server,
                              const float* params_stack,
                              const float* weights_dev, float* round_accum,
                              long long P, int K, hipStream_t s);

void launch_w2_layouts(const float* w2, int K, float* w2t, float* w2rot,
                       hipStream_t s);
void launch_conv2_fwd_mfma(const float* a1, const float* w2t,
                           const float* b2, int bs, int K, float* r2,
                           hipStream_t s);
void launch_conv2_bwd_x_mfma(const float* dz2, const float* w2rot,
                             const float* a1, int bs, int K, float* dz1,
                             hipStream_t s);
void launch_conv2_bwd_w_mfma(const float* dz2, const float* a1, int bs,
                             int K, float* slab, float* dw2, float* db2,
                             hipStream_t s);
void launch_fc1_fwd_mfma(const float* a2, const float* w3, const float* b3,
                         int bs, int K, float p2, unsigned long long seed,
                         unsigned long long offset, float* slab, float* z3,
                         float* a3, unsigned char* m3, hipStream_t s);
void launch_fc1_bwd_w_mfma(const float* dz3, const float* a2, int bs, int K,
                           float* dw3, float* db3, hipStream_t s);
void launch_fc1_bwd_x_mfma(const float* dz3, const float* w3, int bs, int K,
                           float* da2, hipStream_t s);
void launch_mfma_bf16_probe(const void* A, const void* B, float* D,
                            hipStream_t s);
void launch_fc1_fwd_mfma_bf16(const float* a2, const float* w3,
                              const float* b3, int bs, int K, float p2,
                              unsigned long long seed,
                              unsigned long long offset, float* slab,
                              float* z3, float* a3, unsigned char* m3,
                              hipStream_t s);
void launch_conv2_fwd_mfma_bf16(const float* a1, const float* w2b2, int bs,
                                int K, float* r2, hipStream_t s);
void launch_conv2_bwd_x_mfma_bf16(const float* dz2, const float* w2,
                                  const float* a1, int bs, int K,
                                  float* w2rotbf, float* dz1, hipStream_t s);
void launch_conv2_bwd_w_mfma_bf16(const float* dz2, const float* a1, int bs,
                                  int K, float* slab, float* dw2, float* db2,
                                  hipStream_t s);

}
```

Baseline: 188.6 rounds/s.

## Fuse conv2 forward with maxpool/dropout and merge several backward kernels

Conv2 forward (fp32 MFMA path) now does the 2x2 maxpool and dropout in its epilogue through LDS, so the full-resolution r2 activation is no longer written and read back. The pooling index now also records the ReLU-positive bit, which lets a new pool/dropout backward kernel rebuild dz2 without reading r2 and reduce the conv2 bias gradient in the same pass. The fc2 backward-x pass is folded into the loss kernel, the acc2k zeroing moves into the gather kernel in place of a memset, and the separate stats kernel launches are dropped. Together these cut kernel launches and global memory traffic. The cost is a heavier conv2 epilogue with extra syncs and a fixed waves-per-EU setting, plus a single block per row doing the fc2 dz3 work.

```diff
diff --git a/msrflute_amd/csrc/bindings.cpp b/msrflute_amd/csrc/bindings.cpp
--- a/msrflute_amd/csrc/bindings.cpp
+++ b/msrflute_amd/csrc/bindings.cpp
@@ -462,6 +462,55 @@
                         b2.data_ptr<float>(), bs, K, r2.data_ptr<float>(),
                         cur_stream());
   return r2;
+}
+
+std::vector<torch::Tensor> dbg_conv2_fwd_pool_mfma(
+    torch::Tensor a1, torch::Tensor w2, torch::Tensor b2, int64_t bs,
+    int64_t K, double p1, torch::Tensor seeds, int64_t offset) {
+  check_flat(a1, "a1"); check_flat(w2, "w2"); check_flat(b2, "b2");
+  TORCH_CHECK(K >= 1 && bs >= 1 && bs <= 32);
+  long long B = K * bs;
+  TORCH_CHECK(w2.numel() == K * 18432 && b2.numel() == K * 64 &&
+              a1.numel() >= B * 21632);
+  TORCH_CHECK(seeds.scalar_type() == torch::kInt64 && seeds.numel() == K,
+              "seeds must be K int64 values");
+  auto seeds_dev = seeds.to(a1.device()).contiguous();
+  auto w2t = torch::empty_like(w2);
+  auto w2rot = torch::empty_like(w2);
+  auto a2 = torch::empty({B * 9216}, a1.options());
+  auto pidx = torch::empty({B * 9216}, a1.options().dtype(torch::kUInt8));
+  auto m2 = torch::empty({B * 9216}, a1.options().dtype(torch::kUInt8));
+  launch_w2_layouts(w2.data_ptr<float>(), (int)K, w2t.data_ptr<float>(),
+                    w2rot.data_ptr<float>(), cur_stream());
+  launch_conv2_fwd_pool_mfma(
+      a1.data_ptr<float>(), w2t.data_ptr<float>(), b2.data_ptr<float>(),
+      (int)bs, (int)K, (float)p1,
+      reinterpret_cast<const long long*>(seeds_dev.data_ptr<int64_t>()),
+      (unsigned long long)offset, a2.data_ptr<float>(),
+      pidx.data_ptr<unsigned char>(), m2.data_ptr<unsigned char>(),
+      cur_stream());
+  return {a2, pidx, m2};
+}
+
+std::vector<torch::Tensor> dbg_pool_drop_bwd_bias(
+    torch::Tensor da2, torch::Tensor pidx, torch::Tensor m2, int64_t bs,
+    int64_t K, double p1) {
+  check_flat(da2, "da2");
+  TORCH_CHECK(K >= 1 && bs >= 1);
+  long long B = K * bs;
+  TORCH_CHECK(da2.numel() == B * 9216);
+  for (const torch::Tensor* t : {&pidx, &m2})
+    TORCH_CHECK(t->is_cuda() && t->is_contiguous() &&
+                t->scalar_type() == torch::kUInt8 &&
+                t->numel() == B * 9216, "pidx / m2 must be uint8 [B*9216]");
+  auto dz2 = torch::empty({B * 36864}, da2.options());
+  auto db2 = torch::empty({K * 64}, da2.options());
+  launch_pool_drop_bwd_bias(da2.data_ptr<float>(),
+                            pidx.data_ptr<unsigned char>(),
+                            m2.data_ptr<unsigned char>(), (int)bs, (int)K,
+                            (float)p1, dz2.data_ptr<float>(),
+                            db2.data_ptr<float>(), cur_stream());
+  return {dz2, db2};
 }
 
 torch::Tensor dbg_conv2_fwd_mfma_bf16(torch::Tensor a1, torch::Tensor w2,
@@ -771,6 +820,8 @@
         py::arg("dz2"), py::arg("a1"), py::arg("B"), py::arg("K") = 1);
   m.def("dbg_fc1_fwd_mfma_bf16", &dbg_fc1_fwd_mfma_bf16);
   m.def("dbg_conv2_fwd_mfma", &dbg_conv2_fwd_mfma);
+  m.def("dbg_conv2_fwd_pool_mfma", &dbg_conv2_fwd_pool_mfma);
+  m.def("dbg_pool_drop_bwd_bias", &dbg_pool_drop_bwd_bias);
   m.def("dbg_conv2_bwd_x_mfma", &dbg_conv2_bwd_x_mfma);
   m.def("dbg_conv2_bwd_w_mfma", &dbg_conv2_bwd_w_mfma,
         py::arg("dz2"), py::arg("a1"), py::arg("B"), py::arg("K") = 1);
diff --git a/msrflute_amd/csrc/fused_cnn.hip b/msrflute_amd/csrc/fused_cnn.hip
--- a/msrflute_amd/csrc/fused_cnn.hip
+++ b/msrflute_amd/csrc/fused_cnn.hip
@@ -78,8 +78,11 @@
                             const long long* __restrict__ order_offs,
                             const long long* __restrict__ counts,
                             int t, int bs, int K,
-                            float* __restrict__ xb, int* __restrict__ yb) {
+                            float* __restrict__ xb, int* __restrict__ yb,
+                            double* __restrict__ acc2k) {
   int G = K * bs;
+  if (blockIdx.x == 0)
+    for (int q = threadIdx.x; q < 2 * K; q += blockDim.x) acc2k[q] = 0.0;
   for (long long i = blockIdx.x * (long long)blockDim.x + threadIdx.x;
        i < (long long)G * 784; i += (long long)gridDim.x * blockDim.x) {
     int g = (int)(i / 784), j = (int)(i % 784);
@@ -153,12 +156,16 @@
 static_assert(24 % C2F_ROWS == 0 && (C2F_ROWS * 24) % 96 == 0 &&
               C2F_CS % 4 == 0 && C2F_CS / 4 <= 64,
               "conv2 fwd slab: 6 m-tiles per block, float4 plane copies");
-__global__ __launch_bounds__(256)
-void k_conv2_fwd_mfma_mb(const float* __restrict__ a1,
-                         const float* __restrict__ w2t_stack,
-                         const float* __restrict__ params, long long P,
-                         long long ob2, int bs, int K,
-                         float* __restrict__ r2) {
+static_assert(C2F_ROWS == 4 && 2 * 64 * 24 <= 32 * C2F_CS,
+              "POOL epilogue: waves 2mh, 2mh+1 own pool row mh of the slab; "
+              "the cell image fits the staging LDS");
+template <bool POOL>
+__device__ __forceinline__ void conv2_fwd_body(
+    const float* __restrict__ a1, const float* __restrict__ w2t_stack,
+    const float* __restrict__ params, long long P, long long ob2, int bs,
+    float* __restrict__ r2, float p1, unsigned long long seed,
+    unsigned long long offset, float* __restrict__ a2,
+    unsigned char* __restrict__ pidx, unsigned char* __restrict__ m2) {
   __shared__ __attribute__((aligned(16))) float lds[32 * C2F_CS];
   long long g = blockIdx.x / C2F_SLABS;
   int sl = blockIdx.x % C2F_SLABS;
@@ -177,8 +184,13 @@
   conv2_tap_offsets(kc, C2F_CS, 26, 1, off);
   #pragma unroll
   for (int i = 0; i < 3; ++i) {
-    int m = (mh * 3 + i) * 16 + il;
-    base[i] = (m / 24) * 26 + m % 24;
+    if (POOL) {
+      int q = il >> 2, e = il & 3;
+      base[i] = (2 * mh + (e >> 1)) * 26 + 2 * (4 * i + q) + (e & 1);
+    } else {
+      int m = (mh * 3 + i) * 16 + il;
+      base[i] = (m / 24) * 26 + m % 24;
+    }
   }
   const float* wp = w2t_stack + (long long)k * 18432 + kc * 64 + nh * 32 + il;
   f32x4 acc[3][2];
@@ -202,21 +214,110 @@
     }
   }
   const float* b2 = params + (long long)k * P + ob2;
+  if (!POOL) {
+    #pragma unroll
+    for (int n = 0; n < 2; ++n) {
+      int co = nh * 32 + n * 16 + il;
+      float bias = b2[co];
+      #pragma unroll
+      for (int i = 0; i < 3; ++i) {
+        int om = sl * (C2F_ROWS * 24) + (mh * 3 + i) * 16 + kc * 4;
+        float4 v;
+        v.x = acc[i][n][0] + bias; v.y = acc[i][n][1] + bias;
+        v.z = acc[i][n][2] + bias; v.w = acc[i][n][3] + bias;
+        v.x = v.x > 0.f ? v.x : 0.f; v.y = v.y > 0.f ? v.y : 0.f;
+        v.z = v.z > 0.f ? v.z : 0.f; v.w = v.w > 0.f ? v.w : 0.f;
+        *reinterpret_cast<float4*>(r2 + (g * 64 + co) * 576 + om) = v;
+      }
+    }
+    return;
+  }
+  float* cmax = lds;
+  int* cidx = reinterpret_cast<int*>(lds + 64 * 24);
+  __syncthreads();
   #pragma unroll
   for (int n = 0; n < 2; ++n) {
     int co = nh * 32 + n * 16 + il;
     float bias = b2[co];
     #pragma unroll
     for (int i = 0; i < 3; ++i) {
-      int om = sl * (C2F_ROWS * 24) + (mh * 3 + i) * 16 + kc * 4;
-      float4 v;
-      v.x = acc[i][n][0] + bias; v.y = acc[i][n][1] + bias;
-      v.z = acc[i][n][2] + bias; v.w = acc[i][n][3] + bias;
-      v.x = v.x > 0.f ? v.x : 0.f; v.y = v.y > 0.f ? v.y : 0.f;
-      v.z = v.z > 0.f ? v.z : 0.f; v.w = v.w > 0.f ? v.w : 0.f;
-      *reinterpret_cast<float4*>(r2 + (g * 64 + co) * 576 + om) = v;
-    }
-  }
+      float v0 = acc[i][n][0] + bias, v1 = acc[i][n][1] + bias;
+      float v2 = acc[i][n][2] + bias, v3 = acc[i][n][3] + bias;
+      v0 = v0 > 0.f ? v0 : 0.f; v1 = v1 > 0.f ? v1 : 0.f;
+      v2 = v2 > 0.f ? v2 : 0.f; v3 = v3 > 0.f ? v3 : 0.f;
+      float m = v0; int idx = 0;
+      if (v1 > m) { m = v1; idx = 1; }
+      if (v2 > m) { m = v2; idx = 2; }
+      if (v3 > m) { m = v3; idx = 3; }
+      int c = co * 24 + mh * 12 + 4 * i + kc;
+      cmax[c] = m;
+      cidx[c] = idx | (m > 0.f ? 4 : 0);
+    }
+  }
+  __syncthreads();
+  float inv_keep = (p1 < 1.f) ? 1.f / (1.f - p1) : 0.f;
+  int b = (int)(g % bs);
+  #pragma unroll 1
+  for (int c = threadIdx.x; c < 64 * 24; c += 256) {
+    int co = c / 24, rem = c % 24;
+    int lc = co * 144 + sl * 24 + rem;
+    long long i = g * 9216 + lc;
+    int li = b * 9216 + lc;
+    float m = cmax[c];
+    unsigned char keep = 1;
+    if (p1 > 0.f) {
+      hiprandStatePhilox4_32_10_t st;
+      hiprand_init(seed, (unsigned long long)(li >> 2), offset, &st);
+      float4 u = hiprand_uniform4(&st);
+      float uu = (li & 3) == 0 ? u.x : (li & 3) == 1 ? u.y
+                 : (li & 3) == 2 ? u.z : u.w;
+      keep = uu >= p1;
+    }
+    pidx[i] = (unsigned char)cidx[c];
+    m2[i] = keep;
+    a2[i] = keep ? m * inv_keep : 0.f;
+  }
+}
+
+__global__ __launch_bounds__(256)
+void k_conv2_fwd_mfma_mb(const float* __restrict__ a1,
+                         const float* __restrict__ w2t_stack,
+                         const float* __restrict__ params, long long P,
+                         long long ob2, int bs, int K,
+                         float* __restrict__ r2) {
+  conv2_fwd_body<false>(a1, w2t_stack, params, P, ob2, bs, r2, 0.f, 0ull,
+                        0ull, nullptr, nullptr, nullptr);
+}
+
+__global__ __launch_bounds__(256)
+__attribute__((amdgpu_waves_per_eu(5, 5)))
+void k_conv2_fwd_pool_mfma_mb(const float* __restrict__ a1,
+                              const float* __restrict__ w2t_stack,
+                              const float* __restrict__ params, long long P,
+                              long long ob2, int bs, int K, float p1,
+                              const long long* __restrict__ seeds,
+                              unsigned long long offset,
+                              float* __restrict__ a2,
+                              unsigned char* __restrict__ pidx,
+                              unsigned char* __restrict__ m2) {
+  int k = (int)(blockIdx.x / C2F_SLABS / bs);
+  conv2_fwd_body<true>(a1, w2t_stack, params, P, ob2, bs, nullptr, p1,
+                       (unsigned long long)seeds[k], offset, a2, pidx, m2);
+}
+
+__global__ __launch_bounds__(256)
+__attribute__((amdgpu_waves_per_eu(5, 5)))
+void k_conv2_fwd_pool_mfma(const float* __restrict__ a1,
+                           const float* __restrict__ w2t_stack,
+                           const float* __restrict__ params, long long P,
+                           long long ob2, int bs, int K, float p1,
+                           unsigned long long seed,
+                           unsigned long long offset,
+                           float* __restrict__ a2,
+                           unsigned char* __restrict__ pidx,
+                           unsigned char* __restrict__ m2) {
+  conv2_fwd_body<true>(a1, w2t_stack, params, P, ob2, bs, nullptr, p1, seed,
+                       offset, a2, pidx, m2);
 }
 
 template <typename Index>
@@ -239,7 +340,7 @@
                : (li & 3) == 2 ? u.z : u.w;
     keep = uu >= p1;
   }
-  pidx[i] = (unsigned char)idx;
+  pidx[i] = (unsigned char)(idx | (m > 0.f ? 4 : 0));
   m2[i] = keep;
   a2[i] = keep ? m * inv_keep : 0.f;
 }
@@ -510,7 +611,9 @@
 __device__ __forceinline__ void fc2_loss_row(
     const float* __restrict__ ap, const float* __restrict__ w4,
     const float* __restrict__ b4, int target, int Bk, int C,
-    float* __restrict__ dl, float* __restrict__ loss, float* sm) {
+    float* __restrict__ dl, float* __restrict__ loss, float* sm,
+    const float* __restrict__ z3r, const unsigned char* __restrict__ m3r,
+    float p2, float* __restrict__ dz3r) {
   for (int j = threadIdx.x; j < C; j += blockDim.x) {
     const float* wp = w4 + (long long)j * 128;
     float s = b4[j];
@@ -525,11 +628,25 @@
     float z = 0.f;
     for (int j = 0; j < C; ++j) { sm[j] = __expf(sm[j] - mx); z += sm[j]; }
     float inv = 1.f / z;
+    float pt = sm[target] * inv;
     for (int j = 0; j < C; ++j) {
       float p = sm[j] * inv;
-      dl[j] = (p - (j == target ? 1.f : 0.f)) / (float)Bk;
-    }
-    atomicAdd(loss, -__logf(fmaxf(sm[target] * inv, 1e-30f)) / (float)Bk);
+      float d = (p - (j == target ? 1.f : 0.f)) / (float)Bk;
+      dl[j] = d;
+      sm[j] = d;
+    }
+    atomicAdd(loss, -__logf(fmaxf(pt, 1e-30f)) / (float)Bk);
+  }
+  __syncthreads();
+  if (threadIdx.x < 128) {
+    int kk = threadIdx.x;
+    float zv = z3r[kk];
+    unsigned char mk = m3r[kk];
+    float s = 0.f;
+    for (int j = 0; j < C; ++j)
+      s = fmaf(sm[j], w4[(long long)j * 128 + kk], s);
+    float gg = (p2 > 0.f) ? (mk ? s * (1.f / (1.f - p2)) : 0.f) : s;
+    dz3r[kk] = zv > 0.f ? gg : 0.f;
   }
 }
 
@@ -538,11 +655,16 @@
                                const float* __restrict__ b4,
                                const int* __restrict__ yb, int B, int C,
                                float* __restrict__ dlogits,
-                               float* __restrict__ loss_acc) {
+                               float* __restrict__ loss_acc,
+                               const float* __restrict__ z3,
+                               const unsigned char* __restrict__ m3,
+                               float p2, float* __restrict__ dz3) {
   extern __shared__ float sm[];
   int b = blockIdx.x;
   fc2_loss_row(a3 + (long long)b * 128, w4, b4, yb[b], B, C,
-               dlogits + (long long)b * C, loss_acc, sm);
+               dlogits + (long long)b * C, loss_acc, sm,
+               z3 + (long long)b * 128, m3 + (long long)b * 128, p2,
+               dz3 + (long long)b * 128);
 }
 
 __global__ void k_fc2_loss_fwd_mb(const float* __restrict__ a3,
@@ -552,7 +674,10 @@
                                   int t, int bs, int K, int C,
                                   const int* __restrict__ yb,
                                   float* __restrict__ dlogits,
-                                  float* __restrict__ loss_out) {
+                                  float* __restrict__ loss_out,
+                                  const float* __restrict__ z3,
+                                  const unsigned char* __restrict__ m3,
+                                  float p2, float* __restrict__ dz3) {
   extern __shared__ float sm[];
   long long g = blockIdx.x;
   int k = (int)(g / bs);
@@ -560,12 +685,13 @@
   if (target < 0) {
     for (int j = threadIdx.x; j < C; j += blockDim.x)
       dlogits[g * C + j] = 0.f;
+    if (threadIdx.x < 128) dz3[g * 128 + threadIdx.x] = 0.f;
     return;
   }
   fc2_loss_row(a3 + g * 128, params + (long long)k * P + ow4,
                params + (long long)k * P + ob4, target,
                mega_Bk(counts, k, t, bs), C, dlogits + g * C, loss_out + k,
-               sm);
+               sm, z3 + g * 128, m3 + g * 128, p2, dz3 + g * 128);
 }
 
 __global__ void k_fc2_bwd_w_mb(const float* __restrict__ dlogits,
@@ -588,29 +714,6 @@
   }
   grads[(long long)k * P + ow4 + i0] = s;
   if (kk == 0) grads[(long long)k * P + ob4 + j] = sb;
-}
-
-__global__ void k_fc2_bwd_x_mb(const float* __restrict__ dlogits,
-                               const float* __restrict__ params, long long P,
-                               long long ow4, const float* __restrict__ z3,
-                               const unsigned char* __restrict__ m3, int bs,
-                               int K, int C, float p2,
-                               float* __restrict__ dz3) {
-  long long total = (long long)K * bs * 128;
-  float inv_keep = 1.f / (1.f - p2);
-  for (long long i = blockIdx.x * (long long)blockDim.x + threadIdx.x;
-       i < total; i += (long long)gridDim.x * blockDim.x) {
-    int kk = (int)(i % 128);
-    long long g = i / 128;
-    int k = (int)(g / bs);
-    const float* w4 = params + (long long)k * P + ow4;
-    const float* dl = dlogits + g * C;
-    float s = 0.f;
-    for (int j = 0; j < C; ++j)
-      s = fmaf(dl[j], w4[(long long)j * 128 + kk], s);
-    float gg = (p2 > 0.f) ? (m3[i] ? s * inv_keep : 0.f) : s;
-    dz3[i] = z3[i] > 0.f ? gg : 0.f;
-  }
 }
 
 #define FC1B_COL(VEC, g, il) ((g) * 16 * (VEC) + (VEC) * (il))
@@ -755,28 +858,65 @@
   else fc1_bwd_x_body<1>(dz, w3, da, bs, col0);
 }
 
-__global__ void k_pool_drop_bwd_mb(const float* __restrict__ da2,
-                                   const unsigned char* __restrict__ pidx,
-                                   const unsigned char* __restrict__ m2,
-                                   const float* __restrict__ r2, int bs,
-                                   int K, float p1,
-                                   float* __restrict__ dz2) {
-  long long total = (long long)K * bs * 9216;
+__device__ __forceinline__ void conv2_bias_block_sum(float s,
+                                                     float* __restrict__ out) {
+  for (int d = 32; d > 0; d >>= 1) s += __shfl_down(s, d, 64);
+  __shared__ float lds[4];
+  if ((threadIdx.x & 63) == 0) lds[threadIdx.x >> 6] = s;
+  __syncthreads();
+  if (threadIdx.x == 0) {
+    float tt = 0.f;
+    for (int q = 0; q < (int)blockDim.x / 64; ++q) tt += lds[q];
+    *out = tt;
+  }
+}
+
+#define PDB_U 9
+__global__ __launch_bounds__(FBLK)
+void k_pool_drop_bwd_bias_mb(const float* __restrict__ da2,
+                             const unsigned char* __restrict__ pidx,
+                             const unsigned char* __restrict__ m2, int bs,
+                             int K, float p1, float* __restrict__ dz2,
+                             float* __restrict__ grads, long long P,
+                             long long ob2) {
+  int k = blockIdx.x / 64;
+  int co = blockIdx.x % 64;
+  int n = bs * 576;
+  bool drop = p1 > 0.f;
   float inv_keep = (p1 < 1.f) ? 1.f / (1.f - p1) : 0.f;
-  for (long long i = blockIdx.x * (long long)blockDim.x + threadIdx.x;
-       i < total; i += (long long)gridDim.x * blockDim.x) {
-    int px = (int)(i % 12), py = (int)((i / 12) % 12);
-    int c = (int)((i / 144) % 64);
-    long long g = i / 9216;
-    float gg = (p1 > 0.f) ? (m2[i] ? da2[i] * inv_keep : 0.f) : da2[i];
-    int idx = pidx[i];
-    long long base = ((g * 64 + c) * 24 + 2 * py) * 24 + 2 * px;
-    #pragma unroll
-    for (int d = 0; d < 4; ++d) {
-      long long o = base + (d >> 1) * 24 + (d & 1);
-      dz2[o] = (d == idx && r2[o] > 0.f) ? gg : 0.f;
-    }
-  }
+  float sc = drop ? inv_keep : 1.f;
+  const long long row0 = (long long)k * bs * 64 + co;
+  float s = 0.f;
+  for (int e0 = threadIdx.x; e0 < n; e0 += PDB_U * FBLK) {
+    float da[PDB_U];
+    unsigned char pi[PDB_U], mk[PDB_U];
+    #pragma unroll
+    for (int u = 0; u < PDB_U; ++u) {
+      int e = e0 + u * FBLK;
+      e = e < n ? e : n - 1;
+      int b = e / 576, o = e % 576;
+      int y = o / 24, x = o % 24;
+      long long cell = (row0 + (long long)b * 64) * 144 + (y >> 1) * 12
+                       + (x >> 1);
+      da[u] = da2[cell];
+      pi[u] = pidx[cell];
+      mk[u] = m2[cell];
+    }
+    #pragma unroll
+    for (int u = 0; u < PDB_U; ++u) {
+      int e = e0 + u * FBLK;
+      int ec = e < n ? e : n - 1;
+      int b = ec / 576, o = ec % 576;
+      int d = ((o / 24) & 1) * 2 + (o & 1);
+      float gg = (drop && !mk[u]) ? 0.f : da[u] * sc;
+      float v = pi[u] == (d | 4) ? gg : 0.f;
+      if (e < n) {
+        dz2[(row0 + (long long)b * 64) * 576 + o] = v;
+        s += v;
+      }
+    }
+  }
+  conv2_bias_block_sum(s, grads + (long long)k * P + ob2 + co);
 }
 
 #define C2W_ROWS 4
@@ -908,15 +1048,7 @@
     int o = t % 576, b = t / 576;
     s += dzk[((long long)b * 64 + co) * 576 + o];
   }
-  for (int d = 32; d > 0; d >>= 1) s += __shfl_down(s, d, 64);
-  __shared__ float lds[4];
-  if ((threadIdx.x & 63) == 0) lds[threadIdx.x >> 6] = s;
-  __syncthreads();
-  if (threadIdx.x == 0) {
-    float tt = 0.f;
-    for (int q = 0; q < (int)blockDim.x / 64; ++q) tt += lds[q];
-    grads[(long long)k * P + ob2 + co] = tt;
-  }
+  conv2_bias_block_sum(s, grads + (long long)k * P + ob2 + co);
 }
 
 #define C2X_MT 128
@@ -1114,6 +1246,12 @@
                               float* __restrict__ stats_out) {
   long long total = (long long)K * P;
   float lr = lr_t[0];
+  if (blockIdx.x == 0)
+    for (int k = threadIdx.x; k < K; k += blockDim.x) {
+      float scale = clip_scale(acc, k, max_norm, eps);
+      stats_out[2 * k] += scale * (float)acc[2 * k];
+      stats_out[2 * k + 1] += scale * scale * (float)acc[2 * k + 1];
+    }
   long long i = blockIdx.x * (long long)blockDim.x + threadIdx.x;
   if (i >= total) return;
   int k = (int)(i / P);
@@ -1129,18 +1267,6 @@
     if constexpr (STORE_G) grads[i] = gv;
     params[i] -= lr * gv;
   }
-}
-
-__global__ void k_stats_mb(const double* __restrict__ acc, int K,
-                           float max_norm, float eps,
-                           float* __restrict__ stats_out) {
-  int k = blockIdx.x * blockDim.x + threadIdx.x;
-  if (k >= K) return;
-  float norm = (float)sqrt(acc[2 * k + 1]);
-  float scale = (max_norm > 0.f && norm > max_norm)
-                    ? max_norm / (norm + eps) : 1.f;
-  stats_out[2 * k] += scale * (float)acc[2 * k];
-  stats_out[2 * k + 1] += scale * scale * (float)acc[2 * k + 1];
 }
 
 __global__ void k_pseudo_grad_mb(float* __restrict__ grads,
@@ -1457,19 +1583,21 @@
       EPOCH_CHK("k_w2rotbf_mb");
       hipLaunchKernelGGL(k_conv2_fwd_mfma_mb_bf16, dim3(B * 9), dim3(FBLK),
                          0, s, ws.a1, params, P, o.w2, o.b2, B, K, ws.r2);
+      EPOCH_CHK("k_conv2_fwd_mfma_mb_bf16");
+      hipLaunchKernelGGL(k_pool_drop_fwd, dim3((B * 9216 + FBLK - 1) / FBLK),
+                         dim3(FBLK), 0, s, ws.r2, B, p1, seed, off, ws.a2,
+                         ws.pidx, ws.m2);
+      EPOCH_CHK("k_pool_drop_fwd");
     } else {
       hipLaunchKernelGGL(k_w2_layouts_mb, dim3((18432 + FBLK - 1) / FBLK),
                          dim3(FBLK), 0, s, params, P, o.w2, K, ws.w2t,
                          ws.w2rot);
       EPOCH_CHK("k_w2_layouts_mb");
-      hipLaunchKernelGGL(k_conv2_fwd_mfma_mb, dim3(B * C2F_SLABS),
-                         dim3(FBLK), 0, s, ws.a1, ws.w2t, params, P, o.b2, B, K, ws.r2);
-    }
-    EPOCH_CHK("k_conv2_fwd_mfma_mb");
-    hipLaunchKernelGGL(k_pool_drop_fwd, dim3((B * 9216 + FBLK - 1) / FBLK),
-                       dim3(FBLK), 0, s, ws.r2, B, p1, seed, off, ws.a2,
-                       ws.pidx, ws.m2);
-    EPOCH_CHK("k_pool_drop_fwd");
+      hipLaunchKernelGGL(k_conv2_fwd_pool_mfma, dim3(B * C2F_SLABS),
+                         dim3(FBLK), 0, s, ws.a1, ws.w2t, params, P, o.b2, B,
+                         K, p1, seed, off, ws.a2, ws.pidx, ws.m2);
+      EPOCH_CHK("k_conv2_fwd_pool_mfma");
+    }
     if (use_bf16) {
       hipLaunchKernelGGL(k_fc1_fwd_mfma_mb_bf16, dim3(FC1B_SPLIT), dim3(FBLK),
                          0, s, ws.a2, params, P, o.w3, B, K, ws.wsl);
@@ -1490,16 +1618,13 @@
     EPOCH_CHK("k_fc1_fwd_reduce");
     hipLaunchKernelGGL(k_fc2_loss_fwd, dim3(B), dim3(FBLK),
                        C * (int)sizeof(float), s, ws.a3, params + o.w4,
-                       params + o.b4, ws.yb, B, C, ws.dlogits, loss_acc);
+                       params + o.b4, ws.yb, B, C, ws.dlogits, loss_acc,
+                       ws.z3, ws.m3, p2, ws.dz3);
     EPOCH_CHK("k_fc2_loss_fwd");
     hipLaunchKernelGGL(k_fc2_bwd_w_mb, dim3((C * 128 + FBLK - 1) / FBLK),
                        dim3(FBLK), 0, s, ws.dlogits, ws.a3, grads, P, o.w4,
                        o.b4, B, K, C);
     EPOCH_CHK("k_fc2_bwd_w_mb");
-    hipLaunchKernelGGL(k_fc2_bwd_x_mb, dim3((B * 128 + FBLK - 1) / FBLK),
-                       dim3(FBLK), 0, s, ws.dlogits, params, P, o.w4, ws.z3,
-                       ws.m3, B, K, C, p2, ws.dz3);
-    EPOCH_CHK("k_fc2_bwd_x_mb");
     hipLaunchKernelGGL(k_fc1_bwd_w_mfma_mb, dim3(144), dim3(FBLK), 0, s,
                        ws.dz3, ws.a2, grads, P, o.w3, grads, P, o.b3, B, K);
     EPOCH_CHK("k_fc1_bwd_w_mfma_mb");
@@ -1507,10 +1632,10 @@
                        dim3(64 * FC1X_WAVES), 0, s,
                        ws.dz3, params, P, o.w3, B, K, ws.da2);
     EPOCH_CHK("k_fc1_bwd_x_mfma_mb");
-    hipLaunchKernelGGL(k_pool_drop_bwd_mb, dim3((B * 9216 + FBLK - 1) / FBLK),
-                       dim3(FBLK), 0, s, ws.da2, ws.pidx, ws.m2, ws.r2, B, K,
-                       p1, ws.dz2);
-    EPOCH_CHK("k_pool_drop_bwd_mb");
+    hipLaunchKernelGGL(k_pool_drop_bwd_bias_mb, dim3(64), dim3(FBLK), 0, s,
+                       ws.da2, ws.pidx, ws.m2, B, K, p1, ws.dz2, grads, P,
+                       o.b2);
+    EPOCH_CHK("k_pool_drop_bwd_bias_mb");
     if (use_bf16) {
       hipLaunchKernelGGL(k_conv2_bwd_w_mfma_mb_bf16, dim3(18 * B), dim3(FBLK),
                          0, s, ws.dz2, ws.a1, B, K, ws.wsl);
@@ -1522,9 +1647,6 @@
     hipLaunchKernelGGL(k_conv2_bwd_w_fold_mb, dim3((18432 + FBLK - 1) / FBLK),
                        dim3(FBLK), 0, s, ws.wsl, grads, P, o.w2, B, K);
     EPOCH_CHK("k_conv2_bwd_w_fold_mb");
-    hipLaunchKernelGGL(k_conv2_bwd_b_mb, dim3(64), dim3(FBLK), 0, s,
-                       ws.dz2, grads, P, o.b2, B, K);
-    EPOCH_CHK("k_conv2_bwd_b_mb");
     if (use_bf16)
       hipLaunchKernelGGL(k_conv2_bwd_x_mfma_mb_bf16, dim3(B * 22), dim3(FBLK),
                          0, s, ws.dz2,
@@ -1610,7 +1732,7 @@
     hipLaunchKernelGGL(k_gather_mb, dim3((G * 784 + FBLK - 1) / FBLK),
                        dim3(FBLK), 0, s, shard_x, shard_y, orders_dev,
                        row_bases_dev, order_offs_dev, counts_dev, t, bs, K,
-                       xb, yb);
+                       xb, yb, acc2k);
     hipLaunchKernelGGL(k_conv1_fwd_mb,
                        dim3((int)(((long long)G * 21632 + FBLK - 1) / FBLK)),
                        dim3(FBLK), 0, s, xb, params_stack, P, o.w1, o.b1,
@@ -1622,18 +1744,19 @@
                          reinterpret_cast<__bf16*>(w2rot_stack));
       hipLaunchKernelGGL(k_conv2_fwd_mfma_mb_bf16, dim3(G * 9), dim3(FBLK),
                          0, s, a1, params_stack, P, o.w2, o.b2, bs, K, r2);
+      hipLaunchKernelGGL(k_pool_drop_fwd_mb,
+                         dim3((int)(((long long)G * 9216 + FBLK - 1) / FBLK)),
+                         dim3(FBLK), 0, s, r2, bs, K, p1, seeds_dev, off,
+                         a2, pidx, m2);
     } else {
       hipLaunchKernelGGL(k_w2_layouts_mb,
                          dim3((int)(((long long)K * 18432 + FBLK - 1) / FBLK)),
                          dim3(FBLK), 0, s, params_stack, P, o.w2, K,
                          w2t_stack, w2rot_stack);
-      hipLaunchKernelGGL(k_conv2_fwd_mfma_mb, dim3(G * C2F_SLABS),
-                         dim3(FBLK), 0, s, a1, w2t_stack, params_stack, P, o.b2, bs, K, r2);
-    }
-    hipLaunchKernelGGL(k_pool_drop_fwd_mb,
-                       dim3((int)(((long long)G * 9216 + FBLK - 1) / FBLK)),
-                       dim3(FBLK), 0, s, r2, bs, K, p1, seeds_dev, off,
-                       a2, pidx, m2);
+      hipLaunchKernelGGL(k_conv2_fwd_pool_mfma_mb, dim3(G * C2F_SLABS),
+                         dim3(FBLK), 0, s, a1, w2t_stack, params_stack, P,
+                         o.b2, bs, K, p1, seeds_dev, off, a2, pidx, m2);
+    }
     if (use_bf16) {
       hipLaunchKernelGGL(k_fc1_fwd_mfma_mb_bf16, dim3(K * 36), dim3(FBLK),
                          0, s, a2, params_stack, P, o.w3, bs, K, slab);
@@ -1653,23 +1776,20 @@
     }
     hipLaunchKernelGGL(k_fc2_loss_fwd_mb, dim3(G), dim3(FBLK),
                        C * (int)sizeof(float), s, a3, params_stack, P, o.w4,
-                       o.b4, counts_dev, t, bs, K, C, yb, dlogits, loss_out);
+                       o.b4, counts_dev, t, bs, K, C, yb, dlogits, loss_out,
+                       z3, m3, p2, dz3);
     int perk_fc2 = (C * 128 + FBLK - 1) / FBLK;
     hipLaunchKernelGGL(k_fc2_bwd_w_mb, dim3(K * perk_fc2), dim3(FBLK), 0, s,
                        dlogits, a3, grads_stack, P, o.w4, o.b4, bs, K, C);
-    hipLaunchKernelGGL(k_fc2_bwd_x_mb,
-                       dim3((int)(((long long)G * 128 + FBLK - 1) / FBLK)),
-                       dim3(FBLK), 0, s, dlogits, params_stack, P, o.w4,
-                       z3, m3, bs, K, C, p2, dz3);
     hipLaunchKernelGGL(k_fc1_bwd_w_mfma_mb, dim3(K * 144), dim3(FBLK), 0, s,
                        dz3, a2, grads_stack, P, o.w3, grads_stack, P, o.b3,
                        bs, K);
     hipLaunchKernelGGL(k_fc1_bwd_x_mfma_mb, dim3(K * FC1X_BLKS),
                        dim3(64 * FC1X_WAVES), 0, s,
                        dz3, params_stack, P, o.w3, bs, K, da2);
-    hipLaunchKernelGGL(k_pool_drop_bwd_mb,
-                       dim3((int)(((long long)G * 9216 + FBLK - 1) / FBLK)),
-                       dim3(FBLK), 0, s, da2, pidx, m2, r2, bs, K, p1, dz2);
+    hipLaunchKernelGGL(k_pool_drop_bwd_bias_mb, dim3(K * 64), dim3(FBLK), 0,
+                       s, da2, pidx, m2, bs, K, p1, dz2, grads_stack, P,
+                       o.b2);
     if (use_bf16) {
       hipLaunchKernelGGL(k_conv2_bwd_w_mfma_mb_bf16, dim3(18 * G), dim3(FBLK),
                          0, s, dz2, a1, bs, K, slab);
@@ -1680,8 +1800,6 @@
     int perk_fold = (18432 + FBLK - 1) / FBLK;
     hipLaunchKernelGGL(k_conv2_bwd_w_fold_mb, dim3(K * perk_fold),
                        dim3(FBLK), 0, s, slab, grads_stack, P, o.w2, bs, K);
-    hipLaunchKernelGGL(k_conv2_bwd_b_mb, dim3(K * 64), dim3(FBLK), 0, s,
-                       dz2, grads_stack, P, o.b2, bs, K);
     if (use_bf16)
       hipLaunchKernelGGL(k_conv2_bwd_x_mfma_mb_bf16, dim3(G * 22), dim3(FBLK),
                          0, s, dz2,
@@ -1692,12 +1810,9 @@
                          dim3(FBLK), 0, s, dz2, w2rot_stack, a1, bs, K, dz1);
     hipLaunchKernelGGL(k_conv1_bwd_w_mb, dim3(K * 32), dim3(1024), 0, s,
                        xb, dz1, grads_stack, P, o.w1, o.b1, bs, K);
-    hipMemsetAsync(acc2k, 0, 2 * K * sizeof(double), s);
     int blocks_per_k = (int)((P + SUMSQ_CHUNK - 1) / SUMSQ_CHUNK);
     hipLaunchKernelGGL(k_sumsq_mb, dim3(K * blocks_per_k), dim3(FBLK), 0, s,
                        grads_stack, P, blocks_per_k, acc2k);
-    hipLaunchKernelGGL(k_stats_mb, dim3((K + 63) / 64), dim3(64), 0, s,
-                       acc2k, K, max_norm, 1e-6f, stats_out);
     hipLaunchKernelGGL(k_clip_sgd_mb<false>, dim3(gkp), dim3(FBLK), 0, s,
                        params_stack, grads_stack, P, K, acc2k, max_norm,
                        1e-6f, lr_t, stats_out);
@@ -1718,8 +1833,6 @@
   int blocks_per_k = (int)((P + SUMSQ_CHUNK - 1) / SUMSQ_CHUNK);
   hipLaunchKernelGGL(k_sumsq_mb, dim3(K * blocks_per_k), dim3(FBLK), 0, s,
                      grads_stack, P, blocks_per_k, acc2k);
-  hipLaunchKernelGGL(k_stats_mb, dim3((K + 63) / 64), dim3(64), 0, s,
-                     acc2k, K, max_norm, 1e-6f, stats_out);
   long long kp = (long long)K * P;
   int gkp = (int)((kp + FBLK - 1) / FBLK); if (gkp > 4096) gkp = 4096;
   hipLaunchKernelGGL(k_clip_sgd_mb<true>, dim3(gkp), dim3(FBLK), 0, s,
@@ -1755,6 +1868,23 @@
                            int bs, int K, float* r2, hipStream_t s) {
   hipLaunchKernelGGL(k_conv2_fwd_mfma_mb, dim3(K * bs * C2F_SLABS),
                      dim3(FBLK), 0, s, a1, w2t, b2, 64LL, 0LL, bs, K, r2);
+}
+void launch_conv2_fwd_pool_mfma(const float* a1, const float* w2t,
+                                const float* b2, int bs, int K, float p1,
+                                const long long* seeds_dev,
+                                unsigned long long offset, float* a2,
+                                unsigned char* pidx, unsigned char* m2,
+                                hipStream_t s) {
+  hipLaunchKernelGGL(k_conv2_fwd_pool_mfma_mb, dim3(K * bs * C2F_SLABS),
+                     dim3(FBLK), 0, s, a1, w2t, b2, 64LL, 0LL, bs, K, p1,
+                     seeds_dev, offset, a2, pidx, m2);
+}
+void launch_pool_drop_bwd_bias(const float* da2, const unsigned char* pidx,
+                               const unsigned char* m2, int bs, int K,
+                               float p1, float* dz2, float* db2,
+                               hipStream_t s) {
+  hipLaunchKernelGGL(k_pool_drop_bwd_bias_mb, dim3(K * 64), dim3(FBLK), 0, s,
+                     da2, pidx, m2, bs, K, p1, dz2, db2, 64LL, 0LL);
 }
 void launch_conv2_bwd_x_mfma(const float* dz2, const float* w2rot,
                              const float* a1, int bs, int K, float* dz1,
diff --git a/msrflute_amd/csrc/launchers.h b/msrflute_amd/csrc/launchers.h
--- a/msrflute_amd/csrc/launchers.h
+++ b/msrflute_amd/csrc/launchers.h
@@ -145,6 +145,16 @@
 void launch_conv2_fwd_mfma(const float* a1, const float* w2t,
                            const float* b2, int bs, int K, float* r2,
                            hipStream_t s);
+void launch_conv2_fwd_pool_mfma(const float* a1, const float* w2t,
+                                const float* b2, int bs, int K, float p1,
+                                const long long* seeds_dev,
+                                unsigned long long offset, float* a2,
+                                unsigned char* pidx, unsigned char* m2,
+                                hipStream_t s);
+void launch_pool_drop_bwd_bias(const float* da2, const unsigned char* pidx,
+                               const unsigned char* m2, int bs, int K,
+                               float p1, float* dz2, float* db2,
+                               hipStream_t s);
 void launch_conv2_bwd_x_mfma(const float* dz2, const float* w2rot,
                              const float* a1, int bs, int K, float* dz1,
                              hipStream_t s);
```

Result: faster. 203.9 rounds/s (median of 6 runs) (+8.1%).
